# cover-vla/cover-vla

Hardware: AMD Instinct MI355X
Metric: candidate actions scored/sec (whole node), OpenVLA-7B N=32, 224^2 RGB (higher is better)
Workload: dtype bf16; 1 GPU; OpenVLA-7B (DINOv2-L+SigLIP-So400m+Llama-2-7B) N=32 = 8 prompts x 4 samples per GPU, 7 action tokens, 1 224x224 RGB frame(s); CoVer verifier SigLIP2-L/16-384 + 3-member ensemble; random-init weights with decision margins (depth-scaled residual projections, unit-scale embeddings, log-normal gains on the action rows of the head: synth.openvla_state(peaked=True)); candidates_total=32, candidates_per_gpu=32, prompts_per_gpu=8, parallelism=candidate-sharded x1 (weak), own_kv=legacy

## Files before the change

cover_vla_amd/_lib.py:

```python
from __future__ import annotations

import ctypes as C
import os

import torch

_HERE = os.path.dirname(os.path.abspath(__file__))
LIB_PATH = os.environ.get("COVER_LIB_PATH") or os.path.join(_HERE, "libcover_hip.so")

c_p = C.c_void_p
c_ll = C.c_longlong
c_i = C.c_int
c_f = C.c_float


class CoverError(RuntimeError):
    pass


class GemmEpi(C.Structure):
    _fields_ = [("bias", c_p), ("residual", c_p), ("layer_scale", c_p), ("ld_residual", c_i), ("residual_f32", c_i),
                ("act", c_i), ("glu", c_i), ("out_f32", c_i), ("out_scale", c_f),
                ("norm_w", c_p), ("norm_out", c_p), ("ld_norm_out", c_i), ("norm_style", c_i), ("norm_w_offset", c_f),
                ("norm_eps", c_f), ("norm_b", c_p), ("w8", c_p), ("w8_scale", c_p), ("a8", c_p), ("a8_scale", c_p), ("ld_a8", c_i), ("ld_norm_out8", c_i),
                ("norm_out8", c_p), ("norm_out8_scale", c_p),
                ("a8_mx", c_p), ("out8", c_p), ("out8_mx", c_p), ("ld_out8", c_i), ("w8_klinear", c_i)]


class KvSegment(C.Structure):
    _fields_ = [("k", c_p), ("vt", c_p),
                ("k_slot_stride", c_ll), ("k_t_stride", c_ll), ("k_h_stride", c_ll),
                ("vt_slot_stride", c_ll), ("vt_h_stride", c_ll), ("vt_d_stride", c_ll),
                ("slot_of_batch", c_p), ("len_of_batch", c_p), ("vis_len", c_p),
                ("len", c_i), ("mask_mode", c_i), ("causal_offset", c_i), ("_pad", c_i)]


class AttnArgs(C.Structure):
    _fields_ = [("q", c_p), ("out", c_p),
                ("q_b_stride", c_ll), ("q_t_stride", c_ll), ("q_h_stride", c_ll),
                ("o_b_stride", c_ll), ("o_t_stride", c_ll), ("o_h_stride", c_ll),
                ("B", c_i), ("Tq", c_i), ("Hq", c_i), ("Hkv", c_i), ("D", c_i), ("scale", c_f),
                ("n_seg", c_i), ("_pad", c_i), ("seg", KvSegment * 3),
                ("state_in_o", c_p), ("state_in_ml", c_p), ("state_out_o", c_p), ("state_out_ml", c_p),
                ("out8", c_p), ("out8_mx", c_p), ("out8_rows", c_i), ("_pad2", c_i)]


class DecodeAttnArgs(C.Structure):
    _fields_ = [("qkv", c_p), ("ld_qkv", c_i), ("n_splits", c_i), ("partial", c_p), ("bias", c_p),
                ("N", c_i), ("H", c_i), ("D", c_i), ("scale", c_f),
                ("positions", c_p), ("cos_table", c_p), ("sin_table", c_p), ("n_pos", c_i), ("rope_mode", c_i),
                ("seg", KvSegment * 3), ("write_t", c_i), ("_pad", c_i), ("out", c_p), ("out_row_stride", c_ll)]


class OwnAttnArgs(C.Structure):
    _fields_ = [("qkv", c_p), ("ld_qkv", c_i), ("N", c_i), ("H", c_i), ("D", c_i), ("scale", c_f),
                ("positions", c_p), ("cos_table", c_p), ("sin_table", c_p), ("n_pos", c_i), ("rope_mode", c_i),
                ("k", c_p), ("v", c_p), ("k_scale", c_p), ("v_scale", c_p), ("fp8", c_i), ("t_cap", c_i),
                ("slot_stride", c_ll), ("slot_of_batch", c_p), ("write_t", c_i), ("_pad", c_i),
                ("state_o", c_p), ("state_ml", c_p)]


class RopeArgs(C.Structure):
    _fields_ = [("qkv", c_p), ("ld_qkv", c_i),
                ("B", c_i), ("T", c_i), ("Hq", c_i), ("Hkv", c_i), ("D", c_i),
                ("positions", c_p), ("cos_table", c_p), ("sin_table", c_p), ("n_pos", c_i),
                ("rope_mode", c_i),
                ("k_cache", c_p), ("k_slot_stride", c_ll), ("k_t_stride", c_ll), ("k_h_stride", c_ll),
                ("vt_cache", c_p), ("vt_slot_stride", c_ll), ("vt_h_stride", c_ll), ("vt_d_stride", c_ll),
                ("slot_of_batch", c_p), ("t_offset_of_batch", c_p), ("t_offset", c_i), ("n_splits", c_i),
                ("partial", c_p), ("bias", c_p)]


class PatchifyArgs(C.Structure):
    _fields_ = [("img", c_p), ("in_u8_hwc", c_i), ("H", c_i), ("W", c_i), ("patch", c_i), ("n_img", c_i),
                ("img_stride", c_ll), ("mul", c_f * 3), ("add", c_f * 3), ("out", c_p), ("ld_out", c_i)]


class GemmF32Args(C.Structure):
    _fields_ = [("A", c_p), ("a_row_stride", c_ll), ("a_k_stride", c_ll),
                ("B", c_p), ("b_row_stride", c_ll), ("b_k_stride", c_ll),
                ("C", c_p), ("c_row_stride", c_ll),
                ("bias", c_p), ("residual", c_p), ("ld_residual", c_ll),
                ("M", c_i), ("N", c_i), ("K", c_i), ("act", c_i), ("alpha", c_f),
                ("batch", c_i), ("a_batch_stride", c_ll), ("b_batch_stride", c_ll), ("c_batch_stride", c_ll),
                ("bias_batch_stride", c_ll)]


class MhaF32Args(C.Structure):
    _fields_ = [("q", c_p), ("q_b_stride", c_ll), ("q_t_stride", c_ll),
                ("k", c_p), ("k_b_stride", c_ll), ("k_t_stride", c_ll),
                ("v", c_p), ("v_b_stride", c_ll), ("v_t_stride", c_ll),
                ("out", c_p), ("o_b_stride", c_ll), ("o_t_stride", c_ll),
                ("key_pad", c_p), ("B", c_i), ("Tq", c_i), ("Tk", c_i), ("H", c_i), ("Dh", c_i), ("scale", c_f)]


class TokenSelectArgs(C.Structure):
    _fields_ = [("logits", c_p), ("ld", c_ll), ("rows", c_i), ("lo", c_i), ("hi", c_i),
                ("uniform", c_p), ("temperature", c_f), ("token_out", c_p), ("logit_out", c_p)]


class TokenSampleArgs(C.Structure):
    _fields_ = [("logits", c_p), ("ld", c_ll), ("rows", c_i), ("lo", c_i), ("hi", c_i),
                ("uniform", c_p), ("temperature", c_f), ("top_k", c_i), ("top_p", c_f),
                ("token_out", c_p), ("logit_out", c_p), ("kept_out", c_p)]


class TokenSampleScoredArgs(C.Structure):
    _fields_ = TokenSampleArgs._fields_ + [("logprob_out", c_p)]

# ... 106 lines not shown
                ("cum_out", c_p), ("step_lp_out", c_p), ("g_out", c_p), ("kappa_out", c_p)]


class Workspace(C.Structure):
    _fields_ = [("ptr", c_p), ("bytes", C.c_size_t)]


class VitLayer(C.Structure):
    _fields_ = [("ln1_w", c_p), ("ln1_b", c_p), ("ln2_w", c_p), ("ln2_b", c_p),
                ("qkv_w", c_p), ("qkv_b", c_p), ("proj_w", c_p), ("proj_b", c_p),
                ("fc1_w", c_p), ("fc1_b", c_p), ("fc2_w", c_p), ("fc2_b", c_p), ("ls1", c_p), ("ls2", c_p)]


class VitDesc(C.Structure):
    _fields_ = [("dim", c_i), ("heads", c_i), ("head_dim_p", c_i), ("mlp_p", c_i), ("n_layers", c_i), ("act", c_i),
                ("ln_eps", c_f), ("attn_scale", c_f), ("layers_host", C.POINTER(VitLayer)),
                ("last_attn_only", c_i), ("_pad", c_i)]


class DecLayer(C.Structure):
    _fields_ = [("in_norm_w", c_p), ("post_norm_w", c_p), ("qkv_w", c_p), ("qkv_b", c_p), ("o_w", c_p),
                ("gate_up_w", c_p), ("down_w", c_p), ("k_cache", c_p), ("vt_cache", c_p),
                ("qkv_w8", c_p), ("qkv_s", c_p), ("o_w8", c_p), ("o_s", c_p), ("gate_up_w8", c_p), ("gate_up_s", c_p),
                ("down_w8", c_p), ("down_s", c_p), ("down_klinear", c_i), ("o_klinear", c_i)]


class DecDesc(C.Structure):
    _fields_ = [("dim", c_i), ("Hq", c_i), ("Hkv", c_i), ("D", c_i), ("mlp", c_i), ("n_layers", c_i), ("act", c_i),
                ("norm_style", c_i), ("norm_eps", c_f), ("norm_w_offset", c_f), ("attn_scale", c_f),
                ("rope_mode", c_i), ("n_pos", c_i), ("_pad", c_i),
                ("cos_table", c_p), ("sin_table", c_p), ("final_norm_w", c_p),
                ("layers_host", C.POINTER(DecLayer))]


class DecGroup(C.Structure):
    _fields_ = [("B", c_i), ("T", c_i), ("positions", c_p), ("n_seg", c_i), ("write_seg", c_i),
                ("segs", KvSegment * 3), ("seg_k_offset", c_ll * 3), ("seg_vt_offset", c_ll * 3),
                ("write_slot_of_batch", c_p), ("write_t_offset_of_batch", c_p),
                ("write_t_offset", c_i), ("seg0_shared", c_i),
                ("own_kv_mode", c_i), ("seg1_group", c_i), ("seg1_slot_of_group", c_p), ("seg1_len_of_group", c_p),
                ("own_region_elems", c_ll)]


class DecPass(C.Structure):
    _fields_ = [("n_groups", c_i), ("final_norm", c_i), ("x_f32", c_p), ("groups", DecGroup * 2)]


_STRUCTS = {
    "cover_gemm_epi": GemmEpi, "cover_kv_segment": KvSegment, "cover_attn_args": AttnArgs,
    "cover_rope_args": RopeArgs, "cover_patchify_args": PatchifyArgs, "cover_gemm_f32_args": GemmF32Args,
    "cover_mha_f32_args": MhaF32Args, "cover_token_select_args": TokenSelectArgs,
    "cover_token_sample_args": TokenSampleArgs, "cover_token_sample_scored_args": TokenSampleScoredArgs,
    "cover_token_logprob_args": TokenLogprobArgs, "cover_token_topn_args": TokenTopnArgs,
    "cover_token_sample_rows_args": TokenSampleRowsArgs, "cover_token_logprob_rows_args": TokenLogprobRowsArgs,
    "cover_token_topn_rows_args": TokenTopnRowsArgs, "cover_token_allow": TokenAllow, "cover_token_ref": TokenRef, "cover_decode_feedback_args": DecodeFeedbackArgs,
    "cover_token_fsm": TokenFsm,
    "cover_score_select_args": ScoreSelectArgs, "cover_prior_select_args": PriorSelectArgs, "cover_augment_args": AugmentArgs,
    "cover_proposal_prior_args": ProposalPriorArgs,
    "cover_beam_merge_args": BeamMergeArgs,
    "cover_kv_gather_slots_args": KvGatherSlotsArgs, "cover_beam_backtrack_args": BeamBacktrackArgs,
    "cover_gumbel_topn_args": GumbelTopnArgs, "cover_beam_merge_gumbel_args": BeamMergeGumbelArgs, "cover_workspace": Workspace, "cover_vit_layer": VitLayer,
    "cover_vit_desc": VitDesc, "cover_dec_layer": DecLayer, "cover_dec_desc": DecDesc, "cover_dec_group": DecGroup,
    "cover_dec_pass": DecPass, "cover_decode_attn_args": DecodeAttnArgs, "cover_own_attn_args": OwnAttnArgs,
}

_P = C.POINTER
SYMBOLS = {
    "cover_abi_version": (c_i, []),
    "cover_last_error": (C.c_char_p, []),
    "cover_device_info": (c_i, [c_i, _P(c_i), _P(C.c_size_t), C.c_char_p, c_i]),
    "cover_packed_weight_bytes": (C.c_size_t, [c_i, c_i]),
    "cover_packed_k": (c_i, [c_i]),
    "cover_pack_weight_bf16": (c_i, [c_p, c_i, c_i, c_i, c_p, c_i, c_p]),
    "cover_packed_weight_fp8_bytes": (C.c_size_t, [c_i, c_i]),
    "cover_quantize_rows_fp8": (c_i, [c_p, c_i, c_i, c_i, c_p, c_p, c_p]),
    "cover_pack_weight_fp8": (c_i, [c_p, c_i, c_p, c_i, c_i, c_p, c_p, c_i, c_p]),
    "cover_quantize_act_fp8": (c_i, [c_p, c_i, c_i, c_i, c_p, c_i, c_p, c_p]),
    "cover_quantize_act_fp8_mx": (c_i, [c_p, c_i, c_i, c_i, c_p, c_i, c_p, c_p]),
    "cover_pack_weight_fp8_klinear": (c_i, [c_p, c_i, c_p, c_i, c_i, c_p, c_p, c_p]),
    "cover_gemm_workspace_bytes": (C.c_size_t, [c_i, c_i, c_i]),
    "cover_gemm_bf16": (c_i, [c_p, c_i, c_p, c_p, c_i, c_i, c_i, c_i, _P(GemmEpi), c_p, C.c_size_t, c_i, c_p]),
    "cover_gemm_plan_counts": (c_i, [C.POINTER(C.c_longlong), c_i, c_i]),
    "cover_gemm_plan": (c_i, [c_p, c_i, c_p, c_p, c_i, c_i, c_i, c_i, _P(GemmEpi), c_p, C.c_size_t, c_i, C.POINTER(c_i)]),
    "cover_gemm_probe": (c_i, [C.POINTER(C.c_ulonglong)]),
    "cover_attention_bf16": (c_i, [_P(AttnArgs), c_p]),
    "cover_attention_plan": (c_i, [_P(AttnArgs), _P(c_i)]),
    "cover_attention_bf16_pair": (c_i, [_P(AttnArgs), _P(AttnArgs), c_p]),
    "cover_attention_pair_plan": (c_i, [_P(AttnArgs), _P(AttnArgs), _P(c_i)]),
    "cover_decode_attention_fused": (c_i, [_P(DecodeAttnArgs), c_p]),
    "cover_decode_own_attention": (c_i, [_P(OwnAttnArgs), c_p]),
    "cover_layernorm_bf16": (c_i, [c_p, c_i, c_p, c_p, c_p, c_i, c_i, c_i, c_f, c_p]),
    "cover_rmsnorm_bf16": (c_i, [c_p, c_i, c_i, c_p, c_f, c_i, c_p, c_i, c_i, c_i, c_f, c_p]),
    "cover_rmsnorm_bf16_q8": (c_i, [c_p, c_i, c_i, c_p, c_f, c_i, c_p, c_i, c_i, c_i, c_f, c_p, c_i, c_p, c_p]),
    "cover_rope_kv_write": (c_i, [_P(RopeArgs), c_p]),
    "cover_rope_kv_write_pair": (c_i, [_P(RopeArgs), _P(RopeArgs), c_p]),
    "cover_embed_gather": (c_i, [c_p, c_i, c_p, c_i, c_f, c_p, c_i, c_p]),
    "cover_patchify": (c_i, [_P(PatchifyArgs), c_p]),
    "cover_copy_rows_bf16": (c_i, [c_p, c_i, c_p, c_i, c_i, c_i, c_p, c_p, c_p]),
    "cover_add_rows_bf16": (c_i, [c_p, c_i, c_p, c_i, c_i, c_i, c_i, c_p]),
    "cover_scale_bf16": (c_i, [c_p, c_i, c_i, c_i, c_f, c_f, c_p]),
    "cover_cast_f32_to_bf16": (c_i, [c_p, c_i, c_p, c_i, c_i, c_i, c_p]),
    "cover_cast_bf16_to_f32": (c_i, [c_p, c_i, c_p, c_i, c_i, c_i, c_p]),
    "cover_gemm_f32": (c_i, [_P(GemmF32Args), c_p]),
    "cover_gemm_f32_plan": (c_i, [_P(GemmF32Args), _P(c_i)]),
    "cover_layernorm_f32": (c_i, [c_p, c_i, c_p, c_p, c_p, c_i, c_i, c_i, c_f, c_p]),
    "cover_layernorm_f32_grouped": (c_i, [c_p, c_i, c_p, c_p, c_p, c_i, c_i, c_i, c_f, c_i, c_ll, c_p]),
    "cover_softmax_rows_f32": (c_i, [c_p, c_i, c_i, c_i, c_f, c_p]),
    "cover_l2norm_rows_f32": (c_i, [c_p, c_i, c_p, c_i, c_i, c_i, c_p]),
    "cover_add_f32": (c_i, [c_p, c_i, c_p, c_i, c_p, c_i, c_i, c_i, c_i, c_p]),
    "cover_xent_diag_f32": (c_i, [c_p, c_i, c_i, c_i, c_p, c_p, c_p]),
    "cover_act_f32": (c_i, [c_p, c_i, c_p, c_i, c_i, c_i, c_i, c_p]),
    "cover_mha_f32": (c_i, [_P(MhaF32Args), c_p]),
    "cover_masked_mean_f32": (c_i, [c_p, c_p, c_p, c_i, c_i, c_i, c_p]),
    "cover_sincos_time_embed": (c_i, [c_p, c_i, c_i, C.c_double, C.c_double, c_p, c_i, c_p]),
    "cover_token_select": (c_i, [_P(TokenSelectArgs), c_p]),
    "cover_token_sample": (c_i, [_P(TokenSampleArgs), c_p]),
    "cover_token_sample_scored": (c_i, [_P(TokenSampleScoredArgs), c_p]),
    "cover_token_logprob": (c_i, [_P(TokenLogprobArgs), c_p]),
    "cover_token_topn": (c_i, [_P(TokenTopnArgs), c_p]),
    "cover_token_sample_rows": (c_i, [_P(TokenSampleRowsArgs), c_p]),
    "cover_token_logprob_rows": (c_i, [_P(TokenLogprobRowsArgs), c_p]),
    "cover_token_topn_rows": (c_i, [_P(TokenTopnRowsArgs), c_p]),
    "cover_token_sample_rows_allowed": (c_i, [_P(TokenSampleRowsArgs), _P(TokenAllow), c_p]),
    "cover_token_logprob_rows_allowed": (c_i, [_P(TokenLogprobRowsArgs), _P(TokenAllow), c_p]),
    "cover_token_topn_rows_allowed": (c_i, [_P(TokenTopnRowsArgs), _P(TokenAllow), c_p]),
    "cover_token_sample_rows_ref": (c_i, [_P(TokenSampleRowsArgs), _P(TokenAllow), _P(TokenRef), c_p]),
    "cover_decode_feedback": (c_i, [_P(DecodeFeedbackArgs), c_p]),
    "cover_decode_feedback_lp2": (c_i, [_P(DecodeFeedbackArgs), c_p, c_p, c_ll, c_p]),
    "cover_decode_feedback_fsm": (c_i, [_P(DecodeFeedbackArgs), _P(TokenFsm), c_p, c_p, c_ll, c_p]),
    "cover_score_select": (c_i, [_P(ScoreSelectArgs), c_p]),
    "cover_group_argmax": (c_i, [c_p, c_i, c_i, c_p, c_p, c_p]),
    "cover_prior_select": (c_i, [_P(PriorSelectArgs), c_p]),
    "cover_augment_tokens": (c_i, [_P(AugmentArgs), c_p]),
    "cover_augment_actions": (c_i, [_P(AugmentArgs), c_p]),
    "cover_proposal_prior_tokens": (c_i, [_P(ProposalPriorArgs), c_p]),
    "cover_proposal_prior_actions": (c_i, [_P(ProposalPriorArgs), c_p]),
    "cover_beam_merge": (c_i, [_P(BeamMergeArgs), c_p]),
    "cover_kv_gather_slots": (c_i, [_P(KvGatherSlotsArgs), c_p]),
    "cover_beam_backtrack": (c_i, [_P(BeamBacktrackArgs), c_p]),
    "cover_gumbel_topn": (c_i, [_P(GumbelTopnArgs), c_p]),
    "cover_beam_merge_gumbel": (c_i, [_P(BeamMergeGumbelArgs), c_p]),
    "cover_tokens_to_histories": (c_i, [c_p, c_i, c_i, c_i, c_p, c_i, c_p, c_i, c_f, c_p, c_p, c_p]),
    "cover_tokens_to_histories_steps": (c_i, [c_p, c_i, c_i, c_i, c_p, c_i, c_p, c_i, c_i, c_f, c_p, c_p, c_p]),
    "cover_actions_to_histories": (c_i, [c_p, c_ll, c_ll, c_i, c_i, c_p, c_p, c_i, c_f, c_p, c_p, c_p]),
    "cover_resample_axis": (c_i, [c_p, c_i, c_p, c_i, c_i, c_i, c_i, c_i, c_i, c_i, c_p, c_p, c_i, c_i, c_p]),
    "cover_u8_hwc_to_f32_chw_norm": (c_i, [c_p, c_p, c_i, c_i, _P(c_f), _P(c_f), c_p]),
    "cover_u8_hwc_to_f32_chw_scale_norm": (c_i, [c_p, c_p, c_i, c_i, c_f, _P(c_f), _P(c_f), c_p]),
    "cover_resize_bilinear_pad_f32": (c_i, [c_p, c_p, c_i, c_i, c_i, c_i, c_i, c_i, c_i, c_i, c_i, c_f, c_p]),
    "cover_vit_workspace_bytes": (C.c_size_t, [_P(VitDesc), c_i, c_i]),
    "cover_vit_forward": (c_i, [_P(VitDesc), c_p, c_i, c_i, c_p, Workspace, c_i, c_p]),
    "cover_decoder_workspace_bytes": (C.c_size_t, [_P(DecDesc), c_i]),
    "cover_decoder_forward": (c_i, [_P(DecDesc), _P(DecPass), c_p, Workspace, c_i, c_p]),
    "cover_graph_begin": (c_i, [c_p]),
    "cover_graph_end": (c_i, [c_p, _P(c_p)]),
    "cover_graph_launch": (c_i, [c_p, c_p]),
    "cover_graph_destroy": (c_i, [c_p]),
    "cover_timer_create": (c_i, [_P(c_p)]),
    "cover_timer_start": (c_i, [c_p, c_p]),
    "cover_timer_stop": (c_i, [c_p, c_p, _P(c_f)]),
    "cover_timer_destroy": (c_i, [c_p]),
    "cover_stream_sync": (c_i, [c_p]),
    "cover_profile_begin": (c_i, [c_i]),
    "cover_profile_end": (c_i, [_P(C.c_double), _P(C.c_longlong), _P(C.c_double)]),
    "cover_profile_end_n": (c_i, [_P(C.c_double), _P(C.c_longlong), _P(C.c_double), c_i]),
    "cover_sizeof": (C.c_size_t, [C.c_char_p]),
}
# ... 38 lines not shown
```

cover_vla_amd/csrc/capi.hip:

```cpp
#include <hip/hip_runtime.h>
#include <stdio.h>
#include <stdlib.h>
#include <string.h>
#include <string>
#include "kernels.h"

static thread_local std::string g_err;
int fail(int code, const char* what, hipError_t e) {
    char buf[512];
    if (e != hipSuccess) snprintf(buf, sizeof buf, "%s: %s", what, hipGetErrorString(e));
    else snprintf(buf, sizeof buf, "%s", what);
    g_err = buf;
    return code;
}
#define ST(s) ((hipStream_t)(s))

extern "C" {

int cover_abi_version(void) { return COVER_ABI_VERSION; }
const char* cover_last_error(void) { return g_err.c_str(); }

int cover_device_info(int dev, int* n_cu, size_t* total_mem, char* name, int name_len) {
    hipDeviceProp_t p;
    HIPCHK(hipGetDeviceProperties(&p, dev), "hipGetDeviceProperties");
    if (n_cu) *n_cu = p.multiProcessorCount;
    if (total_mem) *total_mem = p.totalGlobalMem;
    if (name && name_len > 0) {
        strncpy(name, p.gcnArchName, name_len - 1);
        name[name_len - 1] = 0;
    }
    return COVER_OK;
}

int cover_packed_k(int K) { return (K + 127) / 128 * 128; }
size_t cover_packed_weight_bytes(int N, int K) {
    return (size_t)((N + 15) / 16) * 16 * (size_t)cover_packed_k(K) * 2;
}
int cover_pack_weight_bf16(const void* W, int ldw, int N, int K, void* Wp, int glu, void* stream) {
    if (!W || !Wp || N <= 0 || K <= 0) return fail(COVER_EINVAL, "cover_pack_weight_bf16: bad arguments");
    if (glu && ((N / 2) % 16 != 0 || (N & 1))) return fail(COVER_EINVAL, "cover_pack_weight_bf16: glu needs N/2 % 16 == 0");
    HIPCHK(launch_pack_weight_bf16((const bf16_t*)W, ldw, N, K, (bf16_t*)Wp, cover_packed_k(K), glu, ST(stream)),
           "pack_weight");
    return COVER_OK;
}
size_t cover_packed_weight_fp8_bytes(int N, int K) { return (size_t)((N + 15) / 16) * 16 * (size_t)cover_packed_k(K); }
int cover_quantize_rows_fp8(const void* W, int ldw, int N, int K, float* scales, void* Wdq, void* stream) {
    if (!W || !scales || !Wdq || N <= 0 || K <= 0) return fail(COVER_EINVAL, "cover_quantize_rows_fp8: bad arguments");
    HIPCHK(launch_quantize_rows_fp8((const bf16_t*)W, ldw, N, K, scales, (bf16_t*)Wdq, ST(stream)), "quantize_rows_fp8");
    return COVER_OK;
}
int cover_pack_weight_fp8(const void* Wdq, int ldw, const float* scales, int N, int K, void* Wq, float* scales_packed, int glu,
                          void* stream) {
    if (!Wdq || !scales || !Wq || !scales_packed || N <= 0 || K <= 0) return fail(COVER_EINVAL, "cover_pack_weight_fp8: bad arguments");
    if (glu && ((N / 2) % 16 != 0 || (N & 1))) return fail(COVER_EINVAL, "cover_pack_weight_fp8: glu needs N/2 % 16 == 0");
    HIPCHK(launch_pack_weight_fp8((const bf16_t*)Wdq, ldw, scales, N, K, (uint8_t*)Wq, scales_packed, cover_packed_k(K), glu, ST(stream)),
           "pack_weight_fp8");
    return COVER_OK;
}
int cover_pack_weight_fp8_klinear(const void* Wdq, int ldw, const float* scales, int N, int K, void* Wq, float* scales_packed, void* stream) {
    if (!Wdq || !scales || !Wq || !scales_packed || N <= 0 || K <= 0) return fail(COVER_EINVAL, "cover_pack_weight_fp8_klinear: bad arguments");
    HIPCHK(launch_pack_weight_fp8((const bf16_t*)Wdq, ldw, scales, N, K, (uint8_t*)Wq, scales_packed, cover_packed_k(K), 0, ST(stream), 1),
           "pack_weight_fp8 (k-linear)");
    return COVER_OK;
}
int cover_quantize_act_fp8_mx(const void* X, int ldx, int M, int K, void* out8, int ld8, void* mx, void* stream) {
    if (!X || !out8 || !mx || M < 0 || K <= 0) return fail(COVER_EINVAL, "cover_quantize_act_fp8_mx: bad arguments");
    HIPCHK(launch_quantize_act_fp8_mx((const bf16_t*)X, ldx, M, K, (uint8_t*)out8, ld8, (uint8_t*)mx, ST(stream)),
           "quantize_act_fp8_mx (ld8 >= padded K, ld8 % 16 == 0, ldx % 8 == 0)");
    return COVER_OK;
}
int cover_quantize_act_fp8(const void* X, int ldx, int M, int K, void* out8, int ld8, float* scales, void* stream) {
    if (!X || !out8 || !scales || M < 0 || K <= 0) return fail(COVER_EINVAL, "cover_quantize_act_fp8: bad arguments");
    HIPCHK(launch_quantize_act_fp8((const bf16_t*)X, ldx, M, K, (uint8_t*)out8, ld8, scales, ST(stream)),
           "quantize_act_fp8 (ld8 >= padded K, ld8 % 16 == 0, ldx % 8 == 0)");
    return COVER_OK;
}
size_t cover_gemm_workspace_bytes(int M, int N, int K) { return gemm_workspace_bytes(M, N, K); }
int cover_gemm_probe(unsigned long long* out) {
    if (!out) return fail(COVER_EINVAL, "cover_gemm_probe: null pointer");
    if (gemm_v3_probe(out) != 0) return fail(COVER_EHIP, "cover_gemm_probe: could not read the probe words");
    return COVER_OK;
}
int cover_gemm_plan_counts(long long* counts, int n, int reset) {
    if (n < 0 || (n > 0 && !counts)) return fail(COVER_EINVAL, "cover_gemm_plan_counts: bad arguments");
    gemm_plan_counts(counts, n, reset);
    return COVER_GEMM_PLANS;
}
static const char* gemm_args_error(const void* A, int lda, const void* Wp, const void* C, int N, int K, const cover_gemm_epi* epi) {
    if (!A || !Wp || !C) return "cover_gemm_bf16: null pointer";
    if (lda % 8) return "cover_gemm_bf16: lda must be a multiple of 8 elements";
    if (lda < cover_packed_k(K)) return "cover_gemm_bf16: lda < padded K";
    if (epi && epi->glu && (N % 32)) return "cover_gemm_bf16: glu needs N % 32 == 0";
    return nullptr;
}
int cover_gemm_plan(const void* A, int lda, const void* Wp, void* C, int ldc, int M, int N, int K,
                    const cover_gemm_epi* epi, void* ws, size_t ws_bytes, int variant, int plan[6]) {
    if (!plan) return fail(COVER_EINVAL, "cover_gemm_plan: null plan");
    if (const char* why = gemm_args_error(A, lda, Wp, C, N, K, epi)) return fail(COVER_EINVAL, why);
    HIPCHK(gemm_plan_query((const bf16_t*)A, lda, (const bf16_t*)Wp, C, ldc, M, N, K, epi, (const float*)ws, ws_bytes, variant, plan), "gemm_plan");
    return COVER_OK;
}
int cover_gemm_bf16(const void* A, int lda, const void* Wp, void* C, int ldc, int M, int N, int K,
                    const cover_gemm_epi* epi, void* ws, size_t ws_bytes, int variant, void* stream) {
    if (const char* why = gemm_args_error(A, lda, Wp, C, N, K, epi)) return fail(COVER_EINVAL, why);
    HIPCHK(launch_gemm_bf16((const bf16_t*)A, lda, (const bf16_t*)Wp, C, ldc, M, N, K, epi, (float*)ws, ws_bytes, variant,
                            ST(stream)),
           "gemm_bf16");
    return COVER_OK;
}

int cover_attention_bf16(const cover_attn_args* a, void* stream) {
    if (!a) return fail(COVER_EINVAL, "cover_attention_bf16: null args");
    HIPCHK(launch_attention_bf16(a, ST(stream)), "attention_bf16 (D must be 64/96/128/256, 1..3 segments)");
    return COVER_OK;
}

int cover_attention_plan(const cover_attn_args* a, int* plan) {
    if (!a || !plan) return fail(COVER_EINVAL, "cover_attention_plan: null pointer");
    HIPCHK(attention_plan(a, plan), "attention_bf16 (D must be 64/96/128/256, 1..3 segments)");
    return COVER_OK;
}
int cover_attention_bf16_pair(const cover_attn_args* a0, const cover_attn_args* a1, void* stream) {
    if (!a0 || !a1) return fail(COVER_EINVAL, "cover_attention_bf16_pair: null args");
    HIPCHK(launch_attention_bf16_pair(a0, a1, ST(stream)), "attention_bf16_pair (D must be 64/96/128/256, 1..3 segments)");
    return COVER_OK;
}
int cover_attention_pair_plan(const cover_attn_args* a0, const cover_attn_args* a1, int* dual) {
    if (!a0 || !a1 || !dual) return fail(COVER_EINVAL, "cover_attention_pair_plan: null pointer");
    HIPCHK(attention_pair_plan(a0, a1, dual), "attention_bf16_pair (D must be 64/96/128/256, 1..3 segments)");
    return COVER_OK;
}
int cover_decode_attention_fused(const cover_decode_attn_args* a, void* stream) {
    if (!a || !a->out || (a->n_splits <= 0 && !a->qkv) || (a->n_splits > 0 && !a->partial))
        return fail(COVER_EINVAL, "cover_decode_attention_fused: null pointer");
    HIPCHK(launch_decode_attention_fused(a, ST(stream)), "decode_attention_fused (D in {64,128}, COVER_MASK_LEN segments, 0 <= write_t < seg[2].len)");
    return COVER_OK;
}

int cover_decode_own_attention(const cover_own_attn_args* a, void* stream) {
    if (!a) return fail(COVER_EINVAL, "cover_decode_own_attention: null args");
    HIPCHK(launch_decode_own_attention(a, ST(stream)), "decode_own_attention (D in {64,128}, 0 <= write_t < t_cap, at most 16 loads per lane per pass)");
    return COVER_OK;
}

int cover_layernorm_bf16(const void* x, int ldx, const float* w, const float* b, void* y, int ldy, int rows, int dim,
                         float eps, void* stream) {
    HIPCHK(launch_layernorm_bf16((const bf16_t*)x, ldx, w, b, (bf16_t*)y, ldy, rows, dim, eps, ST(stream)), "layernorm_bf16");
    return COVER_OK;
}
int cover_rmsnorm_bf16(const void* x, int x_f32, int ldx, const float* w, float w_offset, int style, void* y, int ldy,
                       int rows, int dim, float eps, void* stream) {
    HIPCHK(launch_rmsnorm(x, x_f32, ldx, w, w_offset, style, (bf16_t*)y, ldy, rows, dim, eps, ST(stream)), "rmsnorm_bf16");
    return COVER_OK;
}
int cover_rmsnorm_bf16_q8(const void* x, int x_f32, int ldx, const float* w, float w_offset, int style, void* y, int ldy,
                          int rows, int dim, float eps, void* q8, int ld8, float* q8s, void* stream) {
    if (!q8 || !q8s) return fail(COVER_EINVAL, "cover_rmsnorm_bf16_q8: null q8 / q8s");
    HIPCHK(launch_rmsnorm(x, x_f32, ldx, w, w_offset, style, (bf16_t*)y, ldy, rows, dim, eps, ST(stream), (uint8_t*)q8, ld8, q8s), "rmsnorm_bf16_q8");
    return COVER_OK;
}
int cover_rope_kv_write(const cover_rope_args* a, void* stream) {
    if (!a) return fail(COVER_EINVAL, "cover_rope_kv_write: null args");
    HIPCHK(launch_rope_kv_write(a, ST(stream)), "rope_kv_write");
    return COVER_OK;
}
int cover_rope_kv_write_pair(const cover_rope_args* a0, const cover_rope_args* a1, void* stream) {
    if (!a0 || !a1) return fail(COVER_EINVAL, "cover_rope_kv_write_pair: null args");
    HIPCHK(launch_rope_kv_write_pair(a0, a1, ST(stream)), "rope_kv_write_pair");
    return COVER_OK;
}
int cover_embed_gather(const void* table, int dim, const int64_t* ids, int n, float scale, void* out, int ldo,
                       void* stream) {
    HIPCHK(launch_embed_gather((const bf16_t*)table, dim, ids, n, scale, (bf16_t*)out, ldo, ST(stream)), "embed_gather");
    return COVER_OK;
}
int cover_patchify(const cover_patchify_args* a, void* stream) {
    if (!a || a->patch <= 0 || a->H % a->patch || a->W % a->patch || a->ld_out < 3 * a->patch * a->patch)
        return fail(COVER_EINVAL, "cover_patchify: bad geometry");
    HIPCHK(launch_patchify(a, ST(stream)), "patchify");
    return COVER_OK;
}
int cover_copy_rows_bf16(const void* src, int ld_src, void* dst, int ld_dst, int rows, int cols, const int* sidx,
// ... 364 lines not shown
```

cover_vla_amd/csrc/gemm_bf16.hip:

```cpp
#include <stdlib.h>
#include <string.h>
#include <atomic>
#include <hip/hip_ext.h>
#include "common.h"
#include "kernels.h"

#ifdef COVER_PC_DEBUG
__device__ unsigned long long g_pc_tl[1024 * 8];
#define PCTL(slot) do { if (threadIdx.x == 0) g_pc_tl[((blockIdx.y * gridDim.x + blockIdx.x) & 1023) * 8 + (slot)] = wall_clock64(); } while (0)
#else
#define PCTL(slot) do { } while (0)
#endif

#include "gemm_common.h"



template <int WM, int WN, bool GLDS, int NST_ = 2, int WGM = 2, int WGN = 2>
__global__ __launch_bounds__(64 * WGM * WGN) void gemm_tiled(const bf16_t* __restrict__ A, int lda,
                                                  const bf16_t* __restrict__ Wp, void* C, int ldc, int M, int N,
                                                  int Kp, EpiDev epi, int tiles_m, int tiles_n, int kt_per,
                                                  float* __restrict__ partial) {
    constexpr int NW = WGM * WGN;
    constexpr int BM_ = WGM * WM * 16, BN_ = WGN * WN * 16;
// ... 567 lines not shown
#pragma unroll
        for (int c = 0; c < 2; ++c)
            if ((int)(threadIdx.x + c * 512) * 8 < N)
#pragma unroll
                for (int i = 0; i < 8; ++i) sum += vals[c][i];
        mean = block_sum_lds(sum, red) / N;
        float q2 = 0.f;
#pragma unroll
        for (int c = 0; c < 2; ++c)
            if ((int)(threadIdx.x + c * 512) * 8 < N)
#pragma unroll
                for (int i = 0; i < 8; ++i) {
                    const float d = vals[c][i] - mean;
                    q2 += d * d;
                }
        rstd = rsqrtf(block_sum_lds(q2, red + 8) / N + epi.norm_eps);
    } else {
        RNT(3);
        rstd = rsqrtf(block_sum_lds(q, red) / N + epi.norm_eps);
        RNT(4);
    }
#pragma unroll
    for (int c = 0; c < 2; ++c) {
        const int n0 = (threadIdx.x + c * 512) * 8;
        if (n0 < N) {
            float o[8];
            const float wv[8] = {nw[c][0].x, nw[c][0].y, nw[c][0].z, nw[c][0].w, nw[c][1].x, nw[c][1].y, nw[c][1].z, nw[c][1].w};
#pragma unroll
            for (int i = 0; i < 8; ++i) {
                const float ww = wv[i];
                if (epi.norm_style == 2) o[i] = (vals[c][i] - mean) * rstd * ww + (epi.norm_b ? epi.norm_b[n0 + i] : 0.f);
                else o[i] = epi.norm_style == 1 ? ww * bfround(vals[c][i] * rstd) : vals[c][i] * rstd * (epi.norm_w_offset + ww);
            }
            uint4 u;
            u.x = pack_bf2(o[0], o[1]); u.y = pack_bf2(o[2], o[3]); u.z = pack_bf2(o[4], o[5]); u.w = pack_bf2(o[6], o[7]);
            *(uint4*)(epi.norm_out + (size_t)m * epi.ld_norm_out + n0) = u;
            if (epi.nq8) {
#pragma unroll
                for (int i = 0; i < 8; ++i) vals[c][i] = bfround(o[i]);
            }
        }
    }
    if (epi.nq8) {
        float mx = 0.f;
#pragma unroll
        for (int c = 0; c < 2; ++c)
            if ((int)(threadIdx.x + c * 512) * 8 < N)
#pragma unroll
                for (int i = 0; i < 8; ++i) mx = fmaxf(mx, fabsf(vals[c][i]));
        mx = wave_max(mx);
        if ((threadIdx.x & 63) == 0) red[8 + (threadIdx.x >> 6)] = mx;
        asm volatile("s_waitcnt lgkmcnt(0)\n\ts_barrier" ::: "memory");
        float t = 0.f;
#pragma unroll
        for (int i = 0; i < 8; ++i) t = fmaxf(t, red[8 + i]);
        const float sc = e4m3_pow2_scale(t), inv = 1.0f / sc;
        if (threadIdx.x == 0) epi.nq8s[m] = sc;
        uint8_t* qrow = epi.nq8 + (size_t)m * epi.ldnq8;
#pragma unroll
        for (int c = 0; c < 2; ++c) {
            const int n0 = (threadIdx.x + c * 512) * 8;
            if (n0 < N) store_q8_chunk(qrow, n0, vals[c], inv);
        }
    }
    RNT(5);
}
__global__ __launch_bounds__(512) void splitk_reduce_norm(const float* __restrict__ partial, int S, bf16_t* C, int ldc, int M,
                                                          int N, EpiDev epi) {
    __shared__ float red[16];
    reduce_norm_row(partial, S, C, ldc, M, N, epi, blockIdx.x, red);
}

__device__ __forceinline__ void slab_store4(float* o, const float (&v)[4], int n, int N) {
    if (n + 3 < N && ((((uintptr_t)o) & 15) == 0)) {
        *(float4*)o = make_float4(v[0], v[1], v[2], v[3]);
    } else {
        for (int e = 0; e < 4; ++e)
            if (n + e < N) o[e] = v[e];
    }
}

template <int MF, int KS, int NBW, bool W8 = false>
__global__ __launch_bounds__(512) void gemm_skinny2(const bf16_t* __restrict__ A, int lda, const bf16_t* __restrict__ Wp,
                                                    float* __restrict__ partial, int M, int N, int Kp, const float* __restrict__ wscale, int kl) {
    constexpr int NG = 8 / KS, KC = 256 * KS, NBPB = NG * NBW;
    extern __shared__ __attribute__((aligned(16))) char smem[];
    const int tid = threadIdx.x, lane = tid & 63;
    const int w = __builtin_amdgcn_readfirstlane(tid >> 6);
    const int ks = w % KS, ng = w / KS;
    const int s = blockIdx.y;
    const int k0 = s * KC;
    const int kc = min(KC, Kp - k0);
    const int K32 = Kp >> 5;
    const int N16 = (N + 15) >> 4;
    const int nb_begin = blockIdx.x * NBPB;
    const int kw0 = ks * 256;
    const int nsteps = max(0, min(8, (kc - kw0) >> 5));
    f32x4 acc[NBW][MF];
#pragma unroll
    for (int i = 0; i < NBW; ++i)
#pragma unroll
        for (int f = 0; f < MF; ++f) acc[i][f] = (f32x4){0.f, 0.f, 0.f, 0.f};
    constexpr int NLD = W8 ? 4 : 8;
    auto wsrc = [&](int nb, int k) -> const u32x4* {
        if constexpr (W8) return (const u32x4*)((const uint8_t*)Wp + ((size_t)nb * (Kp >> 6) + (k >> 6)) * 1024) + lane;
        else return (const u32x4*)(Wp + ((size_t)nb * K32 + (k >> 5)) * 512) + lane;
    };
    u32x4 buf[2][NLD];
    auto load8 = [&](u32x4(&dst)[NLD], int i) {
        int nb = nb_begin + ng + NG * i;
        nb = nb < N16 ? nb : N16 - 1;
        const u32x4* src = wsrc(nb, k0 + kw0);
        if (nsteps == 8) {
#pragma unroll
            for (int u = 0; u < NLD; ++u) dst[u] = __builtin_nontemporal_load(src + u * 64);
        } else {
#pragma unroll
            for (int u = 0; u < NLD; ++u)
                if (u * (8 / NLD) < nsteps) dst[u] = __builtin_nontemporal_load(src + u * 64);
        }
    };
    constexpr int NFR = (KC / 32) * MF;
    bool items_done = false;
    if (kc == KC && nsteps == 8 && NBW > 1) {
        constexpr int XL = NFR / 8;
        uint4 xr[XL];
        const int rr = lane & 15, gg = lane >> 4;
#pragma unroll
        for (int j = 0; j < XL; ++j) {
            const int fi = j * 8 + w, kst = fi / MF, f = fi - kst * MF;
            int row = f * 16 + rr;
            row = row < M ? row : M - 1;
            xr[j] = *(const uint4*)(A + (size_t)row * lda + k0 + x_run_k<W8>(kst, gg, kl));
        }
#pragma unroll
        for (int i = 0; i < 2; ++i) {
            int nb = nb_begin + ng + NG * i;
            nb = nb < N16 ? nb : N16 - 1;
            const u32x4* src = wsrc(nb, k0 + kw0);
#pragma unroll
            for (int u = 0; u < NLD; ++u) buf[i][u] = __builtin_nontemporal_load(src + u * 64);
        }
#pragma unroll
        for (int j = 0; j < XL; ++j) *(uint4*)(smem + (j * 8 + w) * 1024 + lane * 16) = xr[j];
        asm volatile("s_waitcnt lgkmcnt(0)\n\ts_barrier" ::: "memory");
#pragma unroll
        for (int i = 0; i < NBW; ++i) {
#pragma unroll
            for (int u = 0; u < 8; ++u) {
                const bf16x8 wf = wfrag<W8>(buf[i & 1], u);
                const int kst = (kw0 >> 5) + u;
#pragma unroll
                for (int f = 0; f < MF; ++f) {
                    const bf16x8 xf = as_bf16x8(*(const uint4*)(smem + ((kst * MF + f) * 64 + lane) * 16));
                    acc[i][f] = __builtin_amdgcn_mfma_f32_16x16x32_bf16(wf, xf, acc[i][f], 0, 0, 0);
                }
            }
            __builtin_amdgcn_sched_barrier(0);
            if (i + 2 < NBW) {
                int nb = nb_begin + ng + NG * (i + 2);
                nb = nb < N16 ? nb : N16 - 1;
                const u32x4* src = wsrc(nb, k0 + kw0);
#pragma unroll
                for (int u = 0; u < NLD; ++u) buf[i & 1][u] = __builtin_nontemporal_load(src + u * 64);
                __builtin_amdgcn_sched_barrier(0);
            }
        }
        items_done = true;
    } else {
        load8(buf[0], 0);
        if (NBW > 1) load8(buf[1], 1);
        {
            const int rr = lane & 15, gg = lane >> 4;
#pragma unroll 4
            for (int fi = w; fi < NFR; fi += 8) {
                const int kst = fi / MF, f = fi - kst * MF;
                const int row = f * 16 + rr, kk = x_run_k<W8>(kst, gg, kl);
                uint4 v = make_uint4(0, 0, 0, 0);
                if (row < M && kk < kc) v = *(const uint4*)(A + (size_t)row * lda + k0 + kk);
                *(uint4*)(smem + fi * 1024 + lane * 16) = v;
            }
        }
        __syncthreads();
    }
    auto comp8 = [&](u32x4(&src)[NLD], f32x4(&a)[MF]) {
        auto step = [&](int u) {
            const bf16x8 wf = wfrag<W8>(src, u);
            const int kst = (kw0 >> 5) + u;
#pragma unroll
            for (int f = 0; f < MF; ++f) {
                const bf16x8 xf = as_bf16x8(*(const uint4*)(smem + ((kst * MF + f) * 64 + lane) * 16));
                a[f] = __builtin_amdgcn_mfma_f32_16x16x32_bf16(wf, xf, a[f], 0, 0, 0);
            }
        };
        if (nsteps == 8) {
#pragma unroll
            for (int u = 0; u < 8; ++u) step(u);
        } else {
#pragma unroll
            for (int u = 0; u < 8; ++u)
                if (u < nsteps) step(u);
        }
    };
    if (!items_done) {
#pragma unroll
        for (int i = 0; i < NBW; ++i) {
            comp8(buf[i & 1], acc[i]);
            if (i + 2 < NBW) load8(buf[i & 1], i + 2);
        }
    }
    constexpr int RB = (8 / MF) < NBW ? (8 / MF) : NBW;
    const int r = lane & 15, g = lane >> 4;
    float* red = (float*)smem;
#pragma unroll
    for (int i0 = 0; i0 < NBW; i0 += RB) {
        __syncthreads();
#pragma unroll
        for (int ii = 0; ii < RB; ++ii)
            if (i0 + ii < NBW) {
#pragma unroll
                for (int f = 0; f < MF; ++f)
#pragma unroll
                    for (int e = 0; e < 4; ++e) red[(((w * RB + ii) * MF + f) * 4 + e) * 64 + lane] = acc[(i0 + ii) < NBW ? (i0 + ii) : 0][f][e];
            }
        __syncthreads();
        constexpr int NFRAG = NG * RB * MF;
        for (int j = w; j < NFRAG; j += 8) {
            const int f = j % MF, ii = (j / MF) % RB, gsel = j / (MF * RB);
            if (i0 + ii >= NBW) continue;
            const int nb = nb_begin + gsel + NG * (i0 + ii);
            float v[4] = {0.f, 0.f, 0.f, 0.f};
#pragma unroll
            for (int kk = 0; kk < KS; ++kk) {
                const int ww = gsel * KS + kk;
#pragma unroll
                for (int e = 0; e < 4; ++e) v[e] += red[(((ww * RB + ii) * MF + f) * 4 + e) * 64 + lane];
            }
            const int m = f * 16 + r, n = nb * 16 + 4 * g;
            if constexpr (W8) {
                const float4 sc = *(const float4*)(wscale + (size_t)(nb < N16 ? nb : N16 - 1) * 16 + 4 * g);
                v[0] *= sc.x; v[1] *= sc.y; v[2] *= sc.z; v[3] *= sc.w;
            }
            if (nb < N16 && m < M && n < N) slab_store4(partial + ((size_t)s * M + m) * N + n, v, n, N);
        }
    }
}

#ifdef COVER_SK_DEBUG
__device__ unsigned long long g_sk_dbg[1024 * 4];
extern "C" int cover_sk_debug(unsigned long long* out) {
    return (int)hipMemcpyFromSymbol(out, HIP_SYMBOL(g_sk_dbg), sizeof(g_sk_dbg));
}
#define SKT(slot) do { if (threadIdx.x == 0) g_sk_dbg[((blockIdx.y * gridDim.x + blockIdx.x) & 1023) * 4 + (slot)] = wall_clock64(); } while (0)
#else
#define SKT(slot) do { } while (0)
#endif
template <int MF, int KS, int NBW, int NBUF, bool W8 = false>
__global__ __launch_bounds__(512) void gemm_skinny3(const bf16_t* __restrict__ A, int lda, const bf16_t* __restrict__ Wp,
                                                    void* C, int ldc, int M, int N, int Kp, EpiDev epi,
                                                    float* __restrict__ partial, int kper, const float* __restrict__ wscale, int kl) {
    SKT(0);
    constexpr int NG = 8 / KS, KC = 256 * KS, NBPB = NG * NBW;
    constexpr int XB = MF * 16 * KC * 2;
    constexpr int XL = XB / (512 * 16);
    extern __shared__ __attribute__((aligned(16))) char smem[];
    const int tid = threadIdx.x, lane = tid & 63;
    const int w = __builtin_amdgcn_readfirstlane(tid >> 6);
    const int ks = w % KS, ng = w / KS;
    const int K32 = Kp >> 5;
    const int N16 = (N + 15) >> 4;
    const int nb_begin = blockIdx.x * NBPB;
    const int kb = blockIdx.y * kper;
    const int ke = min(Kp, kb + kper);
    const int nchunks = (ke - kb + KC - 1) / KC;
    const int kw0 = ks * 256;
    f32x4 acc[NBW][MF];
#pragma unroll
    for (int i = 0; i < NBW; ++i)
#pragma unroll
        for (int f = 0; f < MF; ++f) acc[i][f] = (f32x4){0.f, 0.f, 0.f, 0.f};

    const int items = nchunks * NBW;
    auto steps_of = [&](int c) { return max(0, min(8, (min(KC, ke - kb - c * KC) - kw0) >> 5)); };
    constexpr int NLD = W8 ? 4 : 8;
    auto wsrc = [&](int nb, int k) -> const u32x4* {
        if constexpr (W8) return (const u32x4*)((const uint8_t*)Wp + ((size_t)nb * (Kp >> 6) + (k >> 6)) * 1024) + lane;
        else return (const u32x4*)(Wp + ((size_t)nb * K32 + (k >> 5)) * 512) + lane;
    };
    u32x4 buf[NBUF][NLD];
    auto load8 = [&](u32x4(&dst)[NLD], int t) {
        const int c = t / NBW, i = t - c * NBW;
        int nb = nb_begin + ng + NG * i;
        nb = nb < N16 ? nb : N16 - 1;
        const int nst = steps_of(c);
        const u32x4* src = wsrc(nb, kb + c * KC + kw0);
        if (nst == 8) {
#pragma unroll
            for (int u = 0; u < NLD; ++u) dst[u] = __builtin_nontemporal_load(src + u * 64);
        } else {
#pragma unroll
            for (int u = 0; u < NLD; ++u)
                if (u * (8 / NLD) < nst) dst[u] = __builtin_nontemporal_load(src + u * 64);
        }
    };
    static_assert(XL * 8 == (KC / 32) * MF, "fragments must split evenly over the waves");
    uint4 xr[XL];
    const int srr = lane & 15, sgg = lane >> 4;
    auto x_load = [&](int c) {
        const int k0 = kb + c * KC, kc = min(KC, ke - k0);
#pragma unroll
        for (int j = 0; j < XL; ++j) {
            const int fi = j * 8 + w, kst = fi / MF, f = fi - kst * MF;
            const int row = f * 16 + srr, kk = x_run_k<W8>(kst, sgg, kl);
            xr[j] = make_uint4(0, 0, 0, 0);
            if (row < M && kk < kc) xr[j] = *(const uint4*)(A + (size_t)row * lda + k0 + kk);
        }
    };
    auto x_write = [&](int b) {
#pragma unroll
        for (int j = 0; j < XL; ++j) *(uint4*)(smem + b * XB + (j * 8 + w) * 1024 + lane * 16) = xr[j];
    };
    auto comp8 = [&](u32x4(&src)[NLD], f32x4(&a)[MF], int c) {
        const int nst = steps_of(c);
        const char* xb = smem + (c & 1) * XB;
        auto step = [&](int u) {
            const bf16x8 wf = wfrag<W8>(src, u);
            const int kst = (kw0 >> 5) + u;
#pragma unroll
            for (int f = 0; f < MF; ++f) {
                const bf16x8 xf = as_bf16x8(*(const uint4*)(xb + ((kst * MF + f) * 64 + lane) * 16));
                a[f] = __builtin_amdgcn_mfma_f32_16x16x32_bf16(wf, xf, a[f], 0, 0, 0);
            }
        };
        if (nst == 8) {
#pragma unroll
            for (int u = 0; u < 8; ++u) step(u);
        } else {
#pragma unroll
            for (int u = 0; u < 8; ++u)
                if (u < nst) step(u);
        }
    };

    if (items >= NBUF && min(KC, ke - kb) == KC) {
        {
#pragma unroll
            for (int j = 0; j < XL; ++j) {
                const int fi = j * 8 + w, kst = fi / MF, f = fi - kst * MF;
                int row = f * 16 + srr;
                row = row < M ? row : M - 1;
                xr[j] = *(const uint4*)(A + (size_t)row * lda + kb + x_run_k<W8>(kst, sgg, kl));
            }
        }
#pragma unroll
// ... 74 lines not shown
    }
    int t = c0 * NBW;
    for (int c = c0; c < nchunks; ++c) {
        if (c + 1 < nchunks) x_load(c + 1);
#pragma unroll
        for (int i = 0; i < NBW; ++i, ++t) {
            comp8(buf[i % NBUF], acc[i], c);
            if (t + NBUF < items) load8(buf[i % NBUF], t + NBUF);
        }
        if (c + 1 < nchunks) {
            x_write((c + 1) & 1);
            asm volatile("s_waitcnt lgkmcnt(0)\n\ts_barrier" ::: "memory");
        }
    }

    SKT(2);
    constexpr int RB = (8 / MF) < NBW ? (8 / MF) : NBW;
    const int r = lane & 15, g = lane >> 4;
    float* red = (float*)smem;
#pragma unroll
    for (int i0 = 0; i0 < NBW; i0 += RB) {
        __syncthreads();
#pragma unroll
        for (int ii = 0; ii < RB; ++ii)
            if (i0 + ii < NBW) {
#pragma unroll
                for (int f = 0; f < MF; ++f)
#pragma unroll
                    for (int e = 0; e < 4; ++e) red[(((w * RB + ii) * MF + f) * 4 + e) * 64 + lane] = acc[(i0 + ii) < NBW ? (i0 + ii) : 0][f][e];
            }
        __syncthreads();
        auto slice_sum = [&](int gsel, int ii, int f, float (&v)[4]) {
#pragma unroll
            for (int e = 0; e < 4; ++e) v[e] = 0.f;
#pragma unroll
            for (int kk = 0; kk < KS; ++kk) {
                const int ww = gsel * KS + kk;
#pragma unroll
                for (int e = 0; e < 4; ++e) v[e] += red[(((ww * RB + ii) * MF + f) * 4 + e) * 64 + lane];
            }
            if constexpr (W8) {
                const int nbs = nb_begin + gsel + NG * (i0 + ii);
                const float4 sc = *(const float4*)(wscale + (size_t)(nbs < N16 ? nbs : N16 - 1) * 16 + 4 * g);
                v[0] *= sc.x; v[1] *= sc.y; v[2] *= sc.z; v[3] *= sc.w;
            }
        };
        if (partial) {
            constexpr int NFRAG = NG * RB * MF;
            for (int j = w; j < NFRAG; j += 8) {
                const int f = j % MF, ii = (j / MF) % RB, gsel = j / (MF * RB);
                if (i0 + ii >= NBW) continue;
                const int nb = nb_begin + gsel + NG * (i0 + ii);
                const int m = f * 16 + r, n = nb * 16 + 4 * g;
                if (nb < N16 && m < M && n < N) {
                    float v[4];
                    slice_sum(gsel, ii, f, v);
                    slab_store4(partial + ((size_t)blockIdx.y * M + m) * N + n, v, n, N);
                }
            }
        } else if (epi.glu) {
            constexpr int NFRAG = RB * MF;
            for (int j = w; j < NFRAG; j += 8) {
                const int f = j % MF, ii = j / MF;
                if (i0 + ii >= NBW) continue;
                const int nb = nb_begin + NG * (i0 + ii);
                const int m = f * 16 + r;
                if (nb + 1 < N16 + (N16 & 1) && nb < N16 && m < M) {
                    float gv[4], uv[4];
                    slice_sum(0, ii, f, gv);
                    slice_sum(1, ii, f, uv);
                    epi_store4_glu(epi, C, ldc, m, (nb >> 1) * 16 + 4 * g, N >> 1, gv, uv);
                }
            }
        } else {
            constexpr int NFRAG = NG * RB * MF;
            for (int j = w; j < NFRAG; j += 8) {
                const int f = j % MF, ii = (j / MF) % RB, gsel = j / (MF * RB);
                if (i0 + ii >= NBW) continue;
                const int nb = nb_begin + gsel + NG * (i0 + ii);
                const int m = f * 16 + r;
                if (nb < N16 && m < M) {
                    float v[4];
                    slice_sum(gsel, ii, f, v);
                    epi_store4(epi, C, ldc, m, nb * 16 + 4 * g, N, v);
                }
            }
        }
    }
    SKT(3);
}

__global__ __launch_bounds__(256) void splitk_reduce(const float* __restrict__ partial, int S, void* C, int ldc, int M,
                                                     int N, EpiDev epi) {
    const int Nout = epi.glu ? (N >> 1) : N;
    const int groups = (Nout + 3) >> 2;
    const long long total = (long long)M * groups;
    for (long long idx = (long long)blockIdx.x * blockDim.x + threadIdx.x; idx < total;
         idx += (long long)gridDim.x * blockDim.x) {
        const int m = (int)(idx / groups);
        const int j0 = (int)(idx - (long long)m * groups) * 4;
        if (epi.glu) {
            const int ng = (j0 >> 4) * 32 + (j0 & 15);
            float gv[4] = {0, 0, 0, 0}, uv[4] = {0, 0, 0, 0};
            for (int s = 0; s < S; ++s) {
                const float* p = partial + ((size_t)s * M + m) * N + ng;
#pragma unroll
                for (int i = 0; i < 4; ++i)
                    if (j0 + i < Nout) {
                        gv[i] += p[i];
                        uv[i] += p[16 + i];
                    }
            }
            epi_store4_glu(epi, C, ldc, m, j0, Nout, gv, uv);
        } else {
            float v[4] = {0, 0, 0, 0};
            const float* p0 = partial + (size_t)m * N + j0;
            const size_t sstride = (size_t)M * N;
            if (j0 + 3 < N && ((((uintptr_t)p0) | (sstride * sizeof(float))) & 15) == 0) {
                int s = 0;
                for (; s + 4 <= S; s += 4) {
                    float4 a[4];
#pragma unroll
                    for (int j = 0; j < 4; ++j) a[j] = *(const float4*)(p0 + (s + j) * sstride);
#pragma unroll
                    for (int j = 0; j < 4; ++j) { v[0] += a[j].x; v[1] += a[j].y; v[2] += a[j].z; v[3] += a[j].w; }
                }
                for (; s < S; ++s) {
                    const float4 a = *(const float4*)(p0 + s * sstride);
                    v[0] += a.x; v[1] += a.y; v[2] += a.z; v[3] += a.w;
                }
            } else {
                for (int s = 0; s < S; ++s) {
                    const float* p = partial + ((size_t)s * M + m) * N + j0;
#pragma unroll
                    for (int i = 0; i < 4; ++i)
                        if (j0 + i < N) v[i] += p[i];
                }
            }
            epi_store4(epi, C, ldc, m, j0, N, v);
        }
    }
}


__global__ void pack_weight(const bf16_t* __restrict__ W, int ldw, int N, int K, bf16_t* __restrict__ Wp, int Kp,
                            int glu) {
    const int K32 = Kp >> 5;
    const int N16 = (N + 15) >> 4;
    const long long total = (long long)N16 * K32 * 64;
    for (long long idx = (long long)blockIdx.x * blockDim.x + threadIdx.x; idx < total;
         idx += (long long)gridDim.x * blockDim.x) {
        const int lane = (int)(idx & 63);
        const long long blk = idx >> 6;
        const int kb = (int)(blk % K32);
        const int nb = (int)(blk / K32);
        int n = nb * 16 + (lane & 15);
        if (glu) {
            const int half = N >> 1;
            const int i = nb >> 1;
            n = ((nb & 1) ? half : 0) + i * 16 + (lane & 15);
            if (i * 16 + (lane & 15) >= half) n = N;
        }
        const int k = kb * 32 + (lane >> 4) * 8;
        bf16_t v[8];
#pragma unroll
        for (int e = 0; e < 8; ++e) v[e] = (n < N && k + e < K) ? W[(size_t)n * ldw + k + e] : (bf16_t)0;
        *(uint4*)(Wp + idx * 8) = *(const uint4*)v;
    }
}

static EpiDev make_epi(const cover_gemm_epi* e) {
    EpiDev d;
    d.bias = e ? e->bias : nullptr;
    d.residual = e ? e->residual : nullptr;
    d.res_f32 = e ? e->residual_f32 : 0;
    d.lscale = e ? e->layer_scale : nullptr;
    d.ldr = e ? e->ld_residual : 0;
    d.act = e ? e->act : 0;
    d.glu = e ? e->glu : 0;
    d.out_f32 = e ? e->out_f32 : 0;
    d.out_scale = e ? e->out_scale : 1.0f;
    if (d.out_scale == 0.0f) d.out_scale = 1.0f;
    d.norm_w = e ? e->norm_w : nullptr;
    d.norm_b = e ? e->norm_b : nullptr;
    d.norm_out = e ? (bf16_t*)e->norm_out : nullptr;
    d.ld_norm_out = e ? e->ld_norm_out : 0;
    d.norm_style = e ? e->norm_style : 0;
    d.norm_w_offset = e ? e->norm_w_offset : 0.f;
    d.norm_eps = e ? e->norm_eps : 0.f;
    d.w8 = e ? (const uint8_t*)e->w8 : nullptr;
    d.w8s = e ? e->w8_scale : nullptr;
    if (!d.w8 || !d.w8s) { d.w8 = nullptr; d.w8s = nullptr; }
    d.a8 = e ? (const uint8_t*)e->a8 : nullptr;
    d.a8s = e ? e->a8_scale : nullptr;
    d.lda8 = e ? e->ld_a8 : 0;
    if (!d.a8 || !d.a8s || !d.w8) { d.a8 = nullptr; d.a8s = nullptr; }
    d.nq8 = e ? (uint8_t*)e->norm_out8 : nullptr;
    d.nq8s = e ? e->norm_out8_scale : nullptr;
    d.ldnq8 = e ? e->ld_norm_out8 : 0;
    if (!d.nq8 || !d.nq8s || !d.norm_out || d.norm_style == 2) { d.nq8 = nullptr; d.nq8s = nullptr; }
    d.w8_kl = (e && d.w8) ? e->w8_klinear : 0;
    d.a8mx = (e && d.w8 && e->a8) ? (const uint8_t*)e->a8_mx : nullptr;
    if (d.a8mx) { d.a8 = (const uint8_t*)e->a8; d.a8s = nullptr; }
    d.o8 = e ? (uint8_t*)e->out8 : nullptr;
    d.o8mx = e ? (uint8_t*)e->out8_mx : nullptr;
    d.ldo8 = e ? e->ld_out8 : 0;
    if (!d.o8 || !d.o8mx) { d.o8 = nullptr; d.o8mx = nullptr; }
    return d;
}

static inline int sk_class(int N, int K) { return 2.0 * (double)N * (double)K >= 16.0e6 ? 0 : 3; }

static Skinny3Plan plan_skinny3(int M, int N, int Kp) {
    Skinny3Plan best;
    best.ok = false;
    best.MF = (M + 15) / 16;
    const int N16 = (N + 15) / 16;
    if (M > 32 || (N16 & 1) || Kp < 2048) return best;
    int best_blocks = 0;
    const int nbws[3] = {4, 3, 2};
    for (int bi = 0; bi < 3; ++bi) {
        const int nbw = nbws[bi];
        const int gx = (N16 + 2 * nbw - 1) / (2 * nbw);
        for (int S = 1; S <= 8; ++S) {
            if ((long long)gx * S > 256) break;
            const int kraw = (Kp + S - 1) / S;
            int kper = (kraw + 1023) / 1024 * 1024;
            if ((long long)kper * (S - 1) >= Kp) kper = (kraw + 255) / 256 * 256;
            if (kper < 2048) break;
            if ((long long)kper * (S - 1) >= Kp) continue;
            const int blocks = gx * S;
            if (blocks > best_blocks) {
                best_blocks = blocks;
                best.ok = true; best.NBW = nbw; best.S = S; best.kper = kper; best.gx = gx;
            }
        }
    }
    if (!best.ok || best_blocks < 190) { best.ok = false; return best; }
    best.lds = (size_t)2 * best.MF * 16 * 1024 * 2;
    best.ws_bytes = best.S > 1 ? (size_t)best.S * M * N * sizeof(float) : 0;
    return best;
}

static SkinnyPlan plan_skinny(int M, int N, int Kp) {
    SkinnyPlan p;
    p.MF = (M + 15) / 16;
    const int N16 = (N + 15) / 16;
    p.nbpb = N16 >= 1024 ? 16 : 8;
    p.gx = (N16 + p.nbpb - 1) / p.nbpb;
    const int kc_max = (64 * 1024) / (p.MF * 16 * 2) / 128 * 128;
    int S = (512 + p.gx - 1) / p.gx;
    int kb = Kp / 128;
    if (S > kb) S = kb;
    if (S < 1) S = 1;
    int KC = ((kb + S - 1) / S) * 128;
    if (KC > kc_max) KC = kc_max;
    p.KC = KC;
    p.S = (Kp + KC - 1) / KC;
    p.lds = (size_t)p.MF * 16 * KC * 2;
    p.ws_bytes = (size_t)p.S * M * N * sizeof(float);
    return p;
}

static Skinny2Plan plan_skinny2(int M, int N, int Kp) {
    Skinny2Plan p;
    p.MF = (M + 15) / 16;
    p.KS = p.MF <= 2 ? 4 : 2;
    const int KC = 256 * p.KS, NG = 8 / p.KS;
    p.S = (Kp + KC - 1) / KC;
    const int N16 = (N + 15) / 16;
    static const char* slots_env = getenv("COVER_SK_SLOTS");
    const int slots = slots_env ? atoi(slots_env) : 512;
    if (p.MF <= 2) {
        const int cand[4] = {2, 3, 4, 6};
        p.NBW = 4;
        bool found = false;
        for (int c = 0; c < 4 && !found; ++c) {
            const long long blocks = (long long)((N16 + NG * cand[c] - 1) / (NG * cand[c])) * p.S;
            if (blocks <= slots) { p.NBW = cand[c]; found = true; }
        }
    } else {
        p.NBW = 2;
    }
    p.gx = (N16 + NG * p.NBW - 1) / (NG * p.NBW);
    const int rb = (8 / p.MF) < p.NBW ? (8 / p.MF) : p.NBW;
    const size_t x = (size_t)p.MF * 16 * KC * 2, red = (size_t)8 * rb * p.MF * 4 * 64 * 4;
    p.lds = x > red ? x : red;
    p.ws_bytes = (size_t)p.S * M * N * sizeof(float);
    return p;
}
// ... 139 lines not shown
    if (mx_any) {
        if (!f8_on) return hipErrorInvalidValue;
        if (pick != TP_PC_256x128 && pick != TP_PC_128x256 && pick != TP_PC_224x128 && pick != TP_PC_128x192 && !(pick == TP_PC_64x128 && epi.a8mx && !epi.o8))
            pick = TP_PC_128x256;
    }
    if (!(f8_on && gemm_fp8_tiled_supported(pick)) && ((pick >= TP_PC_128x128 && pick <= TP_PC_128x192) || pick == TP_PC_64x128_S3)) pick = (variant == 2 || pick == TP_PC_64x128_S3) ? TP_64x128 : TP_128x128;
    if (variant == 2 && pick > TP_64x64) pick = TP_128x128;
    const bool f8 = f8_on && gemm_fp8_tiled_supported(pick);
    const TileCfg cd = k_tiles[pick];
    const int bm = cd.wm * cd.wgm * 16, bn = cd.wn * cd.wgn * 16;
    p.pick = pick;
    p.tiles_m = (M + bm - 1) / bm;
    p.tiles_n = (N + bn - 1) / bn;
    const int nk_total = Kp / BK;
    int S = 1;
    if (S_forced > 0 && !force) {
        S = S_forced;
    } else if (ws != nullptr) {
        while ((long long)p.tiles_m * p.tiles_n * S < 192 && S < 8 && nk_total / (S * 2) >= 8 && (size_t)(S * 2) * M * N * sizeof(float) <= ws_bytes)
            S *= 2;
        static const char* split_env = getenv("COVER_TILE_SPLIT");
        if (split_env && atoi(split_env) >= 1 && (size_t)atoi(split_env) * M * N * sizeof(float) <= ws_bytes) S = atoi(split_env);
    }
    if (epi.o8) S = 1;
    const int nst = variant == 2 ? 2 : cd.nst;
    p.lds = (size_t)nst * (bm + bn) * BK * 2;
    p.block = 64 * cd.wgm * cd.wgn;
    p.slot = pick;
    if (f8) {
        if (epi.lda8 < Kp || (epi.lda8 & 15)) return hipErrorInvalidValue;
        static const char* v3f8_env = getenv("COVER_V3_F8");
        const bool v3f8 = !(v3f8_env && v3f8_env[0] == '0') && (size_t)M * epi.lda8 + 4096 < ((size_t)1 << 31);
        p.kind = v3f8 && f8_self_loading(pick) ? GK_F8_V3 : GK_F8_PC;
        if (mx_any && p.kind != GK_F8_V3 && !(pick == TP_PC_64x128 && epi.a8mx && !epi.o8)) return hipErrorInvalidValue;
        if (epi.a8mx) p.lds += p.kind == GK_F8_V3 ? 3 * 1024 : 4 * 256;
        if (p.kind == GK_F8_PC) p.block += 256;
        p.slot = PLAN_FP8;
        const int nk8 = Kp / 128;
        p.kt_per = (nk8 + S - 1) / S;
        p.S = (nk8 + p.kt_per - 1) / p.kt_per;
        return hipSuccess;
    }
    p.kt_per = (nk_total + S - 1) / S;
    p.S = (nk_total + p.kt_per - 1) / p.kt_per;
    if (pick >= TP_V3_224x192) {
        if ((size_t)M * lda * 2 + 4096 >= ((size_t)1 << 31)) return hipErrorInvalidValue;
        p.kind = GK_V3;
        if (pick == TP_V3K_224x96) p.block *= 2;
    } else if (pick == TP_PC_64x128) {
        p.kind = GK_TILED_PC;
        p.block += 256;
    } else {
        p.kind = GK_TILED;
    }
    return hipSuccess;
}

static hipError_t plan_gemm(GemmPlan& p, int lda, const void* C, int ldc, int M, int N, int K, const EpiDev& epi, const float* ws, size_t ws_bytes,
                            int variant, bool want_slabs) {
    p = GemmPlan{};
    p.kind = GK_NONE; p.slot = -1; p.pick = -1;
    if (M <= 0 || N <= 0) return hipSuccess;
    const int Kp = (K + 127) / 128 * 128;
    if (variant == 0) variant = (M <= 64 && ws != nullptr) ? 3 : 1;
    const bool mx_any = epi.a8mx != nullptr || epi.o8 != nullptr;
    if (mx_any) {
        if (variant != 1 || !epi.a8 || !epi.w8 || M <= 64 || (size_t)M * epi.lda8 + 4096 >= ((size_t)1 << 31)) return hipErrorInvalidValue;
        if (epi.a8mx && (!epi.w8_kl || epi.glu)) return hipErrorInvalidValue;
        if (epi.o8 && (!epi.glu || (epi.act != ACT_SILU && epi.act != ACT_GELU_TANH) || ((N / 2) % 32) != 0 || epi.ldo8 < N / 2 || (epi.ldo8 & 15) || epi.out_f32))
            return hipErrorInvalidValue;
        if (epi.o8 && ((((uintptr_t)C) & 15) || (ldc % 8))) return hipErrorInvalidValue;
    }
    if (epi.w8_kl && epi.a8 && !epi.a8mx && M > 64) return hipErrorInvalidValue;
    hipError_t e;
    if (variant == 3 || variant == 6) e = plan_streaming(p, M, N, Kp, ws, ws_bytes, variant == 6, false);
    else if (variant == 5) {
        if (M > 64) return hipErrorInvalidValue;
        p.p1 = plan_skinny(M, N, Kp);
        if (ws == nullptr || ws_bytes < p.p1.ws_bytes) return hipErrorInvalidValue;
        p.kind = GK_SKINNY; p.slot = PLAN_SKINNY; p.S = p.p1.S; p.lds = p.p1.lds;
        e = hipSuccess;
    } else e = plan_tiles(p, lda, M, N, Kp, epi, ws, ws_bytes, variant, mx_any);
    if (e != hipSuccess) return e;
    const bool want_norm = epi.norm_w != nullptr && epi.norm_out != nullptr;
    const bool streaming = p.kind == GK_SKINNY || p.kind == GK_SKINNY2 || p.kind == GK_SKINNY3;
    const bool split = streaming ? !(p.kind == GK_SKINNY3 && p.S == 1) : p.S > 1;
    const bool norm_fusable = want_norm && !epi.glu && !epi.out_f32 && (N % 8) == 0 && N <= 8192 && (ldc % 8) == 0 && (epi.ld_norm_out % 8) == 0 &&
                              (((uintptr_t)epi.norm_w) & 15) == 0;
    p.rcls = streaming ? 5 : p.kind == GK_F8_PC || p.kind == GK_F8_V3 ? 9 : (double)N * (double)Kp >= 16.0e6 ? 8 : 6;
    if (!split) p.done = GD_NONE;
    else if (!streaming && want_slabs && !epi.residual && !epi.lscale && epi.act == ACT_NONE && epi.out_scale == 1.0f && !epi.glu && !epi.norm_out)
        p.done = GD_SLABS;
    else p.done = norm_fusable ? GD_REDUCE_NORM : GD_REDUCE;
    p.norm_launch = want_norm && p.done != GD_REDUCE_NORM;
    return hipSuccess;
}

hipError_t gemm_plan_query(const bf16_t* A, int lda, const bf16_t* Wp, const void* C, int ldc, int M, int N, int K, const cover_gemm_epi* epi_in,
                           const float* ws, size_t ws_bytes, int variant, int* plan) {
    GemmPlan p;
    const hipError_t e = plan_gemm(p, lda, C, ldc, M, N, K, make_epi(epi_in), ws, ws_bytes, variant, false);
    if (e != hipSuccess) return e;
    const int out[6] = {p.slot, p.pick, p.kind == GK_F8_V3 ? 1 : 0, p.S, p.done == GD_NONE ? 0 : p.done == GD_REDUCE ? 1 : 2, p.norm_launch ? 1 : 0};
    for (int i = 0; i < 6; ++i) plan[i] = out[i];
    return hipSuccess;
}

static hipError_t run_norm(const EpiDev& epi, void* C, int ldc, int M, int Nout, hipStream_t st) {
    if (epi.norm_style == 2)
        return launch_layernorm_bf16((const bf16_t*)C, ldc, epi.norm_w, epi.norm_b, epi.norm_out, epi.ld_norm_out, M, Nout, epi.norm_eps, st);
    return launch_rmsnorm(C, 0, ldc, epi.norm_w, epi.norm_w_offset, epi.norm_style, epi.norm_out, epi.ld_norm_out, M, Nout, epi.norm_eps, st,
                          epi.nq8, epi.ldnq8, epi.nq8s);
}

static hipError_t complete_splitk(const GemmPlan& p, const EpiDev& epi, const float* ws, void* C, int ldc, int M, int N, hipStream_t st) {
    hipError_t e = hipSuccess;
    if (p.done == GD_REDUCE_NORM) {
        e = launch_kernel<splitk_reduce_norm>(p.rcls, 0.0, dim3(M), dim3(512), 0, st, ws, p.S, (bf16_t*)C, ldc, M, N, epi);
    } else if (p.done == GD_REDUCE) {
        const int Nout = epi.glu ? N / 2 : N;
        const long long total = (long long)M * ((Nout + 3) / 4);
        int rb = (int)((total + 255) / 256);
        if (rb > 2048) rb = 2048;
        e = launch_kernel<splitk_reduce>(p.rcls, 0.0, dim3(rb), dim3(256), 0, st, ws, p.S, C, ldc, M, N, epi);
    }
    if (e == hipSuccess && p.done != GD_NONE) e = hipGetLastError();
    if (e == hipSuccess && p.norm_launch) e = run_norm(epi, C, ldc, M, epi.glu ? N / 2 : N, st);
    return e;
}

static hipError_t launch_skinny2(const Skinny2Plan& p, const bf16_t* A, int lda, const bf16_t* Wp, float* ws, int M, int N, int K, int Kp,
                                 const uint8_t* w8, const float* w8s, int kl, hipStream_t st) {
    const dim3 grid(p.gx, p.S), block(512);
    plan_hit(PLAN_SKINNY2);
#define SK2(MF_, KS_, NBW_, W8_) launch_kernel<gemm_skinny2<MF_, KS_, NBW_, W8_>>(sk_class(N, K), (W8_ ? 1.0 : 2.0) * (double)N * (double)K, grid, block, p.lds, st, \
                                                                                   A, lda, W8_ ? (const bf16_t*)w8 : Wp, ws, M, N, Kp, w8s, kl)
    hipError_t e;
    if (w8 && w8s && p.MF <= 2) {
        if (p.MF == 1) e = p.NBW == 6 ? SK2(1, 4, 6, true) : p.NBW == 4 ? SK2(1, 4, 4, true) : p.NBW == 3 ? SK2(1, 4, 3, true) : SK2(1, 4, 2, true);
        else e = p.NBW == 6 ? SK2(2, 4, 6, true) : p.NBW == 4 ? SK2(2, 4, 4, true) : p.NBW == 3 ? SK2(2, 4, 3, true) : SK2(2, 4, 2, true);
    } else {
        if (p.MF == 1) e = p.NBW == 6 ? SK2(1, 4, 6, false) : p.NBW == 4 ? SK2(1, 4, 4, false) : p.NBW == 3 ? SK2(1, 4, 3, false) : SK2(1, 4, 2, false);
        else if (p.MF == 2) e = p.NBW == 6 ? SK2(2, 4, 6, false) : p.NBW == 4 ? SK2(2, 4, 4, false) : p.NBW == 3 ? SK2(2, 4, 3, false) : SK2(2, 4, 2, false);
        else if (p.MF == 3) e = SK2(3, 2, 2, false);
        else e = SK2(4, 2, 2, false);
    }
#undef SK2
    if (e == hipSuccess) e = hipGetLastError();
    return e;
}

static hipError_t launch_skinny3(const Skinny3Plan& p, const bf16_t* A, int lda, const bf16_t* Wp, void* C, int ldc, int M, int N,
                                 int Kp, const EpiDev& epi, float* partial, hipStream_t st) {
    const dim3 grid(p.gx, p.S), block(512);
    plan_hit(PLAN_SKINNY3);
#define SK3(MF_, NBW_, W8_) launch_kernel<gemm_skinny3<MF_, 4, NBW_, NBW_, W8_>>(sk_class(N, Kp), (W8_ ? 1.0 : 2.0) * (double)N * (double)Kp, grid, block, p.lds, st, \
                                                                                  A, lda, W8_ ? (const bf16_t*)epi.w8 : Wp, C, ldc, M, N, Kp, epi, partial, p.kper, epi.w8s, epi.w8_kl)
    hipError_t e;
    if (epi.w8) {
        if (p.MF == 1) e = p.NBW == 4 ? SK3(1, 4, true) : p.NBW == 3 ? SK3(1, 3, true) : SK3(1, 2, true);
        else e = p.NBW == 4 ? SK3(2, 4, true) : p.NBW == 3 ? SK3(2, 3, true) : SK3(2, 2, true);
    } else {
        if (p.MF == 1) e = p.NBW == 4 ? SK3(1, 4, false) : p.NBW == 3 ? SK3(1, 3, false) : SK3(1, 2, false);
        else e = p.NBW == 4 ? SK3(2, 4, false) : p.NBW == 3 ? SK3(2, 3, false) : SK3(2, 2, false);
    }
#undef SK3
    if (e == hipSuccess) e = hipGetLastError();
    return e;
}

static hipError_t launch_tiles(const GemmPlan& p, const bf16_t* A, int lda, const bf16_t* Wp, void* C, int ldc, int M, int N, int K, int Kp,
                               const EpiDev& epi, float* partial, int variant, hipStream_t st) {
    const int tcls = (double)N * (double)Kp >= 16.0e6 ? 4 : 1;
    const double twork = 2.0 * (double)M * (double)N * (double)K;
    plan_hit(p.slot);
    if (p.kind == GK_F8_PC || p.kind == GK_F8_V3) return launch_gemm_fp8_tiled(p, epi, C, ldc, M, N, Kp, partial, twork, st);
    if (p.kind == GK_V3) {
        if (p.S == 1 && epi.out_f32 && !epi.bias && !epi.residual && !epi.lscale && epi.act == ACT_NONE && epi.out_scale == 1.0f && !epi.glu &&
            !epi.norm_out && ldc == N)
            partial = (float*)C;
        return launch_gemm_v3(p, A, lda, Wp, C, ldc, M, N, Kp, epi, partial, tcls, twork, st);
    }
    const dim3 grid(p.tiles_m * p.tiles_n, p.S), block(p.block);
#define T(KFN) launch_kernel<KFN>(tcls, twork, grid, block, p.lds, st, A, lda, Wp, C, ldc, M, N, Kp, epi, p.tiles_m, p.tiles_n, p.kt_per, partial)
    hipError_t e;
    if (p.kind == GK_TILED_PC) {
        e = T((gemm_tiled_pc<2, 4, 4, 4>));
    } else if (variant == 2) {
        e = p.pick == TP_128x128 ? T((gemm_tiled<4, 4, false, 2, 2, 2>)) : p.pick == TP_64x128 ? T((gemm_tiled<2, 4, false, 2, 2, 2>)) : T((gemm_tiled<2, 2, false, 2, 2, 2>));
    } else {
        switch (p.pick) {
            case TP_128x128: e = T((gemm_tiled<4, 4, true, 2, 2, 2>)); break;
            case TP_64x128: e = T((gemm_tiled<2, 4, true, 2, 2, 2>)); break;
            case TP_64x64: e = T((gemm_tiled<2, 2, true, 3, 2, 2>)); break;
            case TP_128x128_S4: e = T((gemm_tiled<4, 4, true, 4, 2, 2>)); break;
            case TP_256x128: e = T((gemm_tiled<4, 4, true, 3, 4, 2>)); break;
            case TP_128x256: e = T((gemm_tiled<4, 4, true, 3, 2, 4>)); break;
            case TP_64x128_S3: e = T((gemm_tiled<2, 4, true, 3, 2, 2>)); break;
            case TP_128x128_S3: e = T((gemm_tiled<4, 4, true, 3, 2, 2>)); break;
            default: e = T((gemm_tiled<2, 4, true, 4, 4, 2>)); break;
        }
    }
#undef T
    if (e == hipSuccess) e = hipGetLastError();
    return e;
}

hipError_t launch_gemm_bf16(const bf16_t* A, int lda, const bf16_t* Wp, void* C, int ldc, int M, int N, int K,
                            const cover_gemm_epi* epi_in, float* ws, size_t ws_bytes, int variant, hipStream_t st, int* splits_out) {
    if (splits_out) *splits_out = 0;
    const EpiDev epi = make_epi(epi_in);
    GemmPlan p;
    hipError_t e = plan_gemm(p, lda, C, ldc, M, N, K, epi, ws, ws_bytes, variant, splits_out != nullptr);
    if (e != hipSuccess || p.kind == GK_NONE) return e;
    const int Kp = (K + 127) / 128 * 128;
    float* partial = p.S > 1 ? ws : nullptr;
    switch (p.kind) {
        case GK_SKINNY3: e = launch_skinny3(p.p3, A, lda, Wp, C, ldc, M, N, Kp, epi, partial, st); break;
        case GK_SKINNY2: e = launch_skinny2(p.p2, A, lda, Wp, ws, M, N, K, Kp, epi.w8, epi.w8s, epi.w8_kl, st); break;
        case GK_SKINNY:
            plan_hit(PLAN_SKINNY);
            switch (p.p1.MF) {
#define SK1(MF_) launch_kernel<gemm_skinny<MF_>>(sk_class(N, K), 2.0 * (double)N * (double)K, dim3(p.p1.gx, p.S), dim3(512), p.lds, st, A, lda, Wp, ws, M, N, Kp, \
                                                 p.p1.KC, p.p1.nbpb)
                case 1: e = SK1(1); break;
                case 2: e = SK1(2); break;
                case 3: e = SK1(3); break;
                default: e = SK1(4); break;
#undef SK1
            }
            if (e == hipSuccess) e = hipGetLastError();
            break;
        default: e = launch_tiles(p, A, lda, Wp, C, ldc, M, N, K, Kp, epi, partial, variant, st); break;
    }
    if (e != hipSuccess) return e;
    if (p.done == GD_SLABS) {
        *splits_out = p.S;
        return e;
    }
    return complete_splitk(p, epi, ws, C, ldc, M, N, st);
}

hipError_t launch_gemm_skinny_partial(const bf16_t* A, int lda, const bf16_t* Wp, float* ws, size_t ws_bytes, int M, int N,
                                      int K, int* S_out, hipStream_t st, const void* w8, const float* w8s) {
    if (M <= 0 || M > 64 || N <= 0) return hipErrorInvalidValue;
    const int Kp = (K + 127) / 128 * 128;
    GemmPlan p = GemmPlan{};
    hipError_t e = plan_streaming(p, M, N, Kp, ws, ws_bytes, false, true);
    if (e != hipSuccess) return e;
    if (p.kind == GK_SKINNY3) {
        EpiDev none = make_epi(nullptr);
        if (w8 && w8s) { none.w8 = (const uint8_t*)w8; none.w8s = w8s; }
        e = launch_skinny3(p.p3, A, lda, Wp, nullptr, 0, M, N, Kp, none, ws, st);
    } else {
        e = launch_skinny2(p.p2, A, lda, Wp, ws, M, N, K, Kp, (const uint8_t*)w8, w8s, 0, st);
    }
    *S_out = p.S;
    return e;
}

__global__ __launch_bounds__(256) void quantize_rows_fp8_k(const bf16_t* __restrict__ W, int ldw, int K, float* __restrict__ scales,
                                                           bf16_t* __restrict__ Wdq) {
    __shared__ float red[16];
    const int n = blockIdx.x;
    const bf16_t* w = W + (size_t)n * ldw;
    float mx = 0.f;
    for (int k = threadIdx.x; k < K; k += blockDim.x) mx = fmaxf(mx, fabsf(bf2f(w[k])));
    mx = block_max(mx, red);
    float s = 1.0f;
    if (mx > 0.f) {
        int e;
        const float f = frexpf(mx / 448.0f, &e);
        s = ldexpf(1.0f, f == 0.5f ? e - 1 : e);
    }
    if (threadIdx.x == 0) scales[n] = s;
    const float inv = 1.0f / s;
    for (int k = threadIdx.x; k < K; k += blockDim.x) {
        const float x = bf2f(w[k]) * inv;
        const int pk = __builtin_amdgcn_cvt_pk_fp8_f32(x, 0.0f, 0, false);
        const f32x2_t back = __builtin_amdgcn_cvt_pk_f32_fp8((uint32_t)pk, false);
        Wdq[(size_t)n * ldw + k] = f2bf(back[0] * s);
    }
}

__global__ void pack_weight_fp8_k(const bf16_t* __restrict__ Wdq, int ldw, const float* __restrict__ scales, int N, int K,
                                  uint8_t* __restrict__ Wq, float* __restrict__ scales_packed, int Kp, int glu, int kl) {
    const int K64 = Kp >> 6;
    const int N16 = (N + 15) >> 4;
    const long long total = (long long)N16 * K64 * 64;
    for (long long idx = (long long)blockIdx.x * blockDim.x + threadIdx.x; idx < total; idx += (long long)gridDim.x * blockDim.x) {
        const int lane = (int)(idx & 63);
        const long long blk = idx >> 6;
        const int kb = (int)(blk % K64);
        const int nb = (int)(blk / K64);
        int n = nb * 16 + (lane & 15);
        if (glu) {
            const int half = N >> 1, i = nb >> 1;
            n = ((nb & 1) ? half : 0) + i * 16 + (lane & 15);
            if (i * 16 + (lane & 15) >= half) n = N;
        }
        const float s = n < N ? scales[n] : 1.0f, inv = 1.0f / s;
        if (kb == 0 && (lane >> 4) == 0) scales_packed[nb * 16 + (lane & 15)] = s;
        uint32_t o[4];
#pragma unroll
        for (int half_ = 0; half_ < 2; ++half_) {
            const int k = kl ? kb * 64 + (lane >> 4) * 16 + half_ * 8 : kb * 64 + half_ * 32 + (lane >> 4) * 8;
            float v[8];
#pragma unroll
            for (int e = 0; e < 8; ++e) v[e] = (n < N && k + e < K) ? bf2f(Wdq[(size_t)n * ldw + k + e]) * inv : 0.f;
            int lo = __builtin_amdgcn_cvt_pk_fp8_f32(v[0], v[1], 0, false);
            lo = __builtin_amdgcn_cvt_pk_fp8_f32(v[2], v[3], lo, true);
            int hi = __builtin_amdgcn_cvt_pk_fp8_f32(v[4], v[5], 0, false);
            hi = __builtin_amdgcn_cvt_pk_fp8_f32(v[6], v[7], hi, true);
            o[2 * half_] = (uint32_t)lo;
            o[2 * half_ + 1] = (uint32_t)hi;
        }
        *(uint4*)(Wq + idx * 16) = make_uint4(o[0], o[1], o[2], o[3]);
    }
}

hipError_t launch_quantize_rows_fp8(const bf16_t* W, int ldw, int N, int K, float* scales, bf16_t* Wdq, hipStream_t st) {
    if (N <= 0) return hipSuccess;
    hipLaunchKernelGGL(quantize_rows_fp8_k, dim3(N), dim3(256), 0, st, W, ldw, K, scales, Wdq);
    return hipGetLastError();
}
hipError_t launch_pack_weight_fp8(const bf16_t* Wdq, int ldw, const float* scales, int N, int K, uint8_t* Wq, float* scales_packed,
                                  int Kpad, int glu, hipStream_t st, int kl) {
    const long long total = (long long)((N + 15) / 16) * (Kpad / 64) * 64;
    int blocks = (int)((total + 255) / 256);
    if (blocks > 65535) blocks = 65535;
    hipLaunchKernelGGL(pack_weight_fp8_k, dim3(blocks), dim3(256), 0, st, Wdq, ldw, scales, N, K, Wq, scales_packed, Kpad, glu, kl);
    return hipGetLastError();
}

hipError_t launch_pack_weight_bf16(const bf16_t* W, int ldw, int N, int K, bf16_t* Wp, int Kpad, int glu,
                                   hipStream_t st) {
    const long long total = (long long)((N + 15) / 16) * (Kpad / 32) * 64;
    int blocks = (int)((total + 255) / 256);
// ... 5 lines not shown
```

cover_vla_amd/csrc/gemm_common.h:

```cpp
#pragma once
#include <type_traits>
#include "common.h"
#include "kernels.h"

#define BK 64
#ifndef PCTL
#define PCTL(slot) do { } while (0)
#endif

struct EpiDev {
    const float* bias;
    const void* residual;
    const float* lscale;
    int ldr, res_f32, act, glu, out_f32;
    float out_scale;
    const float* norm_w;
    const float* norm_b;
    bf16_t* norm_out;
    int ld_norm_out, norm_style;
    float norm_w_offset, norm_eps;
    const uint8_t* w8;
    const float* w8s;
    const uint8_t* a8;
    const float* a8s;
    int lda8;
    uint8_t* nq8;
    float* nq8s;
    int ldnq8;
    int w8_kl;
    const uint8_t* a8mx;
    uint8_t* o8;
    uint8_t* o8mx;
    int ldo8;
};

__device__ __forceinline__ void store_q8_chunk(uint8_t* row, int k, const float (&v)[8], float inv) {
    int lo = __builtin_amdgcn_cvt_pk_fp8_f32(v[0] * inv, v[1] * inv, 0, false);
    lo = __builtin_amdgcn_cvt_pk_fp8_f32(v[2] * inv, v[3] * inv, lo, true);
    int hi = __builtin_amdgcn_cvt_pk_fp8_f32(v[4] * inv, v[5] * inv, 0, false);
    hi = __builtin_amdgcn_cvt_pk_fp8_f32(v[6] * inv, v[7] * inv, hi, true);
    *(uint2*)(row + (k >> 6) * 64 + ((k >> 3) & 3) * 16 + ((k >> 5) & 1) * 8) = make_uint2((uint32_t)lo, (uint32_t)hi);
}
__device__ __forceinline__ float e4m3_pow2_scale(float mx) {
    float s = 1.0f;
    if (mx > 0.f) {
        int e;
        const float f = frexpf(mx / 448.0f, &e);
        s = ldexpf(1.0f, f == 0.5f ? e - 1 : e);
    }
    return s;
}
__device__ __forceinline__ uint32_t mx_quant_chunk(const float (&v)[8], uint2& q) {
    float mx = 0.f;
#pragma unroll
    for (int e = 0; e < 8; ++e) mx = fmaxf(mx, fabsf(v[e]));
    mx = fmaxf(mx, __builtin_bit_cast(float, __builtin_amdgcn_update_dpp(0, __builtin_bit_cast(int, mx), 0xB1, 0xf, 0xf, true)));
    mx = fmaxf(mx, __builtin_bit_cast(float, __builtin_amdgcn_update_dpp(0, __builtin_bit_cast(int, mx), 0x4E, 0xf, 0xf, true)));
    const float s = fmaxf(e4m3_pow2_scale(mx), 1.1754943508222875e-38f);
    const float inv = 1.0f / s;
    int lo = __builtin_amdgcn_cvt_pk_fp8_f32(v[0] * inv, v[1] * inv, 0, false);
    lo = __builtin_amdgcn_cvt_pk_fp8_f32(v[2] * inv, v[3] * inv, lo, true);
    int hi = __builtin_amdgcn_cvt_pk_fp8_f32(v[4] * inv, v[5] * inv, 0, false);
    hi = __builtin_amdgcn_cvt_pk_fp8_f32(v[6] * inv, v[7] * inv, hi, true);
    q = make_uint2((uint32_t)lo, (uint32_t)hi);
    return (__builtin_bit_cast(uint32_t, s) >> 23) & 0xffu;
}

__device__ __forceinline__ void epi_value4(const EpiDev& e, int m, int n0, int N, float v[4]) {
    const bool full = (n0 + 3 < N);
    if (full) {
        float b[4] = {0.f, 0.f, 0.f, 0.f}, ls[4] = {1.f, 1.f, 1.f, 1.f}, r[4] = {0.f, 0.f, 0.f, 0.f};
        if (e.bias) {
#pragma unroll
            for (int i = 0; i < 4; ++i) b[i] = e.bias[n0 + i];
        }
        if (e.lscale) {
#pragma unroll
            for (int i = 0; i < 4; ++i) ls[i] = e.lscale[n0 + i];
        }
        if (e.residual) {
            if (e.res_f32) {
                const float* rp = (const float*)e.residual + (size_t)m * e.ldr + n0;
#pragma unroll
                for (int i = 0; i < 4; ++i) r[i] = rp[i];
            } else {
                const bf16_t* rp = (const bf16_t*)e.residual + (size_t)m * e.ldr + n0;
#pragma unroll
                for (int i = 0; i < 4; ++i) r[i] = bf2f(rp[i]);
            }
        }
#pragma unroll
        for (int i = 0; i < 4; ++i) {
            float x = v[i];
            if (e.bias) x += b[i];
            x = bfround(x);
            if (e.act != ACT_NONE) x = bfround(act_apply_bf16(x, e.act));
            if (e.lscale) x = bfround(x * ls[i]);
            if (e.residual) x = x + r[i];
            if (e.out_scale != 1.0f) x *= e.out_scale;
            v[i] = x;
        }
        return;
    }
#pragma unroll
    for (int i = 0; i < 4; ++i) {
        float x = v[i];
        if (e.bias && (full || n0 + i < N)) x += e.bias[n0 + i];
        x = bfround(x);
        if (e.act != ACT_NONE) x = bfround(act_apply_bf16(x, e.act));
        v[i] = x;
    }
    if (e.lscale) {
#pragma unroll
        for (int i = 0; i < 4; ++i)
            if (full || n0 + i < N) v[i] = bfround(v[i] * e.lscale[n0 + i]);
    }
    if (e.residual) {
        if (e.res_f32) {
            const float* r = (const float*)e.residual + (size_t)m * e.ldr + n0;
#pragma unroll
            for (int i = 0; i < 4; ++i)
                if (full || n0 + i < N) v[i] = v[i] + r[i];
        } else {
            const bf16_t* r = (const bf16_t*)e.residual + (size_t)m * e.ldr + n0;
#pragma unroll
            for (int i = 0; i < 4; ++i)
                if (full || n0 + i < N) v[i] = v[i] + bf2f(r[i]);
        }
    }
    if (e.out_scale != 1.0f) {
#pragma unroll
        for (int i = 0; i < 4; ++i) v[i] *= e.out_scale;
    }
}
__device__ __forceinline__ bool epi_is_plain(const EpiDev& e) {
    return !e.bias && !e.residual && !e.lscale && e.act == ACT_NONE && e.out_scale == 1.0f;
}
__device__ __forceinline__ void epi_put4(const EpiDev& e, void* C, int ldc, int m, int n0, int N, const float v[4]) {
    if (n0 >= N) return;
    const bool full = (n0 + 3 < N);
    if (e.out_f32) {
        float* o = (float*)C + (size_t)m * ldc + n0;
        if (full && ((((uintptr_t)o) & 15) == 0)) {
            *(float4*)o = make_float4(v[0], v[1], v[2], v[3]);
        } else {
#pragma unroll
            for (int i = 0; i < 4; ++i)
                if (n0 + i < N) o[i] = v[i];
        }
    } else {
        bf16_t* o = (bf16_t*)C + (size_t)m * ldc + n0;
        if (full && ((((uintptr_t)o) & 7) == 0)) {
            uint2 p;
            p.x = pack_bf2(v[0], v[1]);
            p.y = pack_bf2(v[2], v[3]);
            *(uint2*)o = p;
        } else {
#pragma unroll
            for (int i = 0; i < 4; ++i)
                if (n0 + i < N) o[i] = f2bf(v[i]);
        }
    }
}

__device__ __forceinline__ void epi_store4(const EpiDev& e, void* C, int ldc, int m, int n0, int N, float v[4]) {
    if (n0 >= N) return;
    const bool full = (n0 + 3 < N);
    epi_value4(e, m, n0, N, v);
    if (e.out_f32) {
        float* o = (float*)C + (size_t)m * ldc + n0;
        if (full && ((((uintptr_t)o) & 15) == 0)) {
            *(float4*)o = make_float4(v[0], v[1], v[2], v[3]);
        } else {
            for (int i = 0; i < 4; ++i)
                if (n0 + i < N) o[i] = v[i];
        }
    } else {
        bf16_t* o = (bf16_t*)C + (size_t)m * ldc + n0;
        if (full && ((((uintptr_t)o) & 7) == 0)) {
            uint2 p;
            p.x = pack_bf2(v[0], v[1]);
            p.y = pack_bf2(v[2], v[3]);
            *(uint2*)o = p;
        } else {
            for (int i = 0; i < 4; ++i)
                if (n0 + i < N) o[i] = f2bf(v[i]);
        }
    }
}

__device__ __forceinline__ void epi_store4_glu(const EpiDev& e, void* C, int ldc, int m, int j0, int Nout, float g[4],
                                               float u[4]) {
    if (j0 >= Nout) return;
    float v[4];
#pragma unroll
    for (int i = 0; i < 4; ++i) {
        float gg = bfround(g[i]), uu = bfround(u[i]);
        gg = bfround(act_apply_bf16(gg, e.act));
        v[i] = bfround(gg * uu);
    }
    if (e.out_f32) {
        float* o = (float*)C + (size_t)m * ldc + j0;
        for (int i = 0; i < 4; ++i)
            if (j0 + i < Nout) o[i] = v[i];
    } else {
        bf16_t* o = (bf16_t*)C + (size_t)m * ldc + j0;
        if (j0 + 3 < Nout && ((((uintptr_t)o) & 7) == 0)) {
            uint2 p;
            p.x = pack_bf2(v[0], v[1]);
            p.y = pack_bf2(v[2], v[3]);
            *(uint2*)o = p;
        } else {
            for (int i = 0; i < 4; ++i)
                if (j0 + i < Nout) o[i] = f2bf(v[i]);
        }
    }
}

template <int WM, int WN, int F>
__device__ __forceinline__ void tiled_epilogue_row(f32x4 (&acc)[WN][WM], const EpiDev& epi, void* C, int ldc, int M, int N, int mw,
                                                   int nw, int r, int g, float* __restrict__ partial) {
    const int m = mw + F * 16 + r;
    if (m < M) {
        if (partial) {
#pragma unroll
            for (int b = 0; b < WN; ++b) {
                const int n = nw + b * 16 + 4 * g;
                if (n < N) {
                    float* o = partial + ((size_t)blockIdx.y * M + m) * N + n;
                    if (n + 3 < N && ((((uintptr_t)o) & 15) == 0)) {
                        *(float4*)o = make_float4(acc[b][F][0], acc[b][F][1], acc[b][F][2], acc[b][F][3]);
                    } else {
                        const float v[4] = {acc[b][F][0], acc[b][F][1], acc[b][F][2], acc[b][F][3]};
#pragma unroll
                        for (int i = 0; i < 4; ++i)
                            if (n + i < N) o[i] = v[i];
                    }
                }
            }
        } else if (epi.glu) {
#pragma unroll
            for (int b = 0; b < WN; b += 2) {
                const int nblk = (nw >> 4) + b;
                float gv[4] = {acc[b][F][0], acc[b][F][1], acc[b][F][2], acc[b][F][3]};
                float uv[4] = {acc[b + 1][F][0], acc[b + 1][F][1], acc[b + 1][F][2], acc[b + 1][F][3]};
                epi_store4_glu(epi, C, ldc, m, (nblk >> 1) * 16 + 4 * g, N >> 1, gv, uv);
            }
        } else {
            float vv[WN][4];
#pragma unroll
            for (int b = 0; b < WN; ++b) {
#pragma unroll
                for (int i = 0; i < 4; ++i) vv[b][i] = acc[b][F][i];
                const int n = nw + b * 16 + 4 * g;
                if (n < N) epi_value4(epi, m, n, N, vv[b]);
            }
#pragma unroll
            for (int b = 0; b < WN; ++b) epi_put4(epi, C, ldc, m, nw + b * 16 + 4 * g, N, vv[b]);
        }
    }
    if constexpr (F + 1 < WM) tiled_epilogue_row<WM, WN, F + 1>(acc, epi, C, ldc, M, N, mw, nw, r, g, partial);
}
template <int WM, int WN>
__device__ __forceinline__ void tiled_epilogue(f32x4 (&acc)[WN][WM], const EpiDev& epi, void* C, int ldc, int M, int N, int mw,
                                               int nw, int r, int g, float* __restrict__ partial) {
    tiled_epilogue_row<WM, WN, 0>(acc, epi, C, ldc, M, N, mw, nw, r, g, partial);
}

template <int WM, int WN, int F>
__device__ __forceinline__ void staged_fill_row(f32x4 (&acc)[WN][WM], char* st, int pitch, int m0, int n0, int mw, int nw, int r, int g,
// ... 217 lines not shown
        } else {
            if (epi.out_f32) {
                const float4 a4 = *(const float4*)(lrow + ch * 16);
                float v[4] = {a4.x, a4.y, a4.z, a4.w};
                epi_value4(epi, m, n0 + ch * 4, N, v);
                *(float4*)dst = make_float4(v[0], v[1], v[2], v[3]);
            } else {
                const float4 a4 = *(const float4*)(lrow + ch * 32), b4 = *(const float4*)(lrow + ch * 32 + 16);
                float v[4] = {a4.x, a4.y, a4.z, a4.w}, w[4] = {b4.x, b4.y, b4.z, b4.w};
                epi_value4(epi, m, n0 + ch * 8, N, v);
                epi_value4(epi, m, n0 + ch * 8 + 4, N, w);
                *(uint4*)dst = make_uint4(pack_bf2(v[0], v[1]), pack_bf2(v[2], v[3]), pack_bf2(w[0], w[1]), pack_bf2(w[2], w[3]));
            }
        }
    }
    }
}

__device__ __forceinline__ void glds16_s(uint32_t voff, const void* sbase, uint32_t lds_wave_base_u32) {
    uint32_t keep;
    asm volatile(
        "s_mov_b32 %0, m0\n\t"
        "s_mov_b32 m0, %3\n\t"
        "s_nop 0\n\t"
        "global_load_lds_dwordx4 %1, %2\n\t"
        "s_mov_b32 m0, %0"
        : "=&s"(keep)
        : "v"(voff), "s"(sbase), "s"(lds_wave_base_u32)
        : "memory");
}

__device__ __forceinline__ void glds4_s(uint32_t voff, const void* sbase, uint32_t lds_wave_base_u32) {
    uint32_t keep;
    asm volatile(
        "s_mov_b32 %0, m0\n\t"
        "s_mov_b32 m0, %3\n\t"
        "s_nop 0\n\t"
        "global_load_lds_dword %1, %2\n\t"
        "s_mov_b32 m0, %0"
        : "=&s"(keep)
        : "v"(voff), "s"(sbase), "s"(lds_wave_base_u32)
        : "memory");
}


enum TilePick {
    TP_128x128 = 0, TP_64x128 = 1, TP_64x64 = 2, TP_128x128_S4 = 3, TP_256x128 = 4, TP_128x256 = 5, TP_128x128_W8 = 6, TP_64x128_S3 = 7,
    TP_128x128_S3 = 8,
    TP_PC_64x128_S3 = 9, TP_PC_64x128 = 10, TP_PC_128x128 = 11, TP_PC_256x128 = 12, TP_PC_128x256 = 13, TP_PC_224x96_W4 = 14,
    TP_PC_224x128 = 15, TP_PC_224x192 = 16, TP_PC_224x96 = 17, TP_PC_128x192 = 18,
    PLAN_SKINNY2 = 19, PLAN_SKINNY3 = 20, PLAN_FP8 = 21, PLAN_SKINNY = 22,
    TP_V3_224x192 = 23, TP_V3_224x128 = 24, TP_V3_256x128 = 25, TP_V3_128x256 = 26, TP_V3_224x96 = 27,
    TP_V3K_224x96 = 30,
};

struct SkinnyPlan {
    int MF, KC, S, nbpb, gx;
    size_t lds, ws_bytes;
};
struct Skinny2Plan {
    int MF, KS, NBW, gx, S;
    size_t lds, ws_bytes;
};
struct Skinny3Plan {
    bool ok;
    int MF, NBW, S, kper, gx;
    size_t lds, ws_bytes;
};

enum GemmKind { GK_NONE, GK_SKINNY, GK_SKINNY2, GK_SKINNY3, GK_TILED, GK_TILED_PC, GK_F8_PC, GK_F8_V3, GK_V3 };
enum GemmDone { GD_NONE = 0, GD_REDUCE = 1, GD_REDUCE_NORM = 2, GD_SLABS = 3 };

struct GemmPlan {
    GemmKind kind;
    int slot;
    int pick;
    int S, kt_per;
    int tiles_m, tiles_n, block;
    size_t lds;
    SkinnyPlan p1;
    Skinny2Plan p2;
    Skinny3Plan p3;
    GemmDone done;
    bool norm_launch;
    int rcls;
};

template <auto kfn, typename... Args>
static inline hipError_t launch_kernel(int cls, double work, dim3 grid, dim3 block, size_t lds, hipStream_t st, Args... args) {
    if (lds > 64 * 1024) {
        static LdsAttrCache c;
        const hipError_t e = lds_attr_160k_cached((const void*)kfn, c);
        if (e != hipSuccess) return e;
    }
    hipEvent_t ea, eb;
    if (prof_enabled() && prof_reserve(cls, work, &ea, &eb) >= 0)
        hipExtLaunchKernelGGL(kfn, grid, block, (uint32_t)lds, st, ea, eb, 0, args...);
    else
        hipLaunchKernelGGL(kfn, grid, block, lds, st, args...);
    return hipSuccess;
}

bool gemm_fp8_tiled_supported(int pick);
hipError_t launch_gemm_fp8_tiled(const GemmPlan& p, const EpiDev& epi, void* C, int ldc, int M, int N, int Kp, float* partial, double prof_work,
                                 hipStream_t st);

hipError_t launch_gemm_v3(const GemmPlan& p, const bf16_t* A, int lda, const bf16_t* Wp, void* C, int ldc, int M, int N, int Kp, const EpiDev& epi,
                          float* partial, int prof_cls, double prof_work, hipStream_t st);
```

cover_vla_amd/csrc/kernels.h:

```cpp
#pragma once
#include <hip/hip_runtime.h>
#include <stdint.h>
#include "../../include/cover_hip.h"

typedef uint16_t bf16_t;

hipError_t launch_gemm_bf16(const bf16_t* A, int lda, const bf16_t* Wp, void* C, int ldc, int M, int N, int K,
                            const cover_gemm_epi* epi, float* splitk_ws, size_t splitk_ws_bytes, int variant,
                            hipStream_t st, int* splits_out = nullptr);
hipError_t launch_gemm_skinny_partial(const bf16_t* A, int lda, const bf16_t* Wp, float* ws, size_t ws_bytes, int M, int N,
                                      int K, int* S_out, hipStream_t st, const void* w8 = nullptr, const float* w8s = nullptr);
#define COVER_GEMM_PLANS 32
hipError_t gemm_plan_query(const bf16_t* A, int lda, const bf16_t* Wp, const void* C, int ldc, int M, int N, int K, const cover_gemm_epi* epi,
                           const float* ws, size_t ws_bytes, int variant, int* plan);
void gemm_plan_counts(long long* out, int n, int reset);
int gemm_v3_probe(unsigned long long* out);
hipError_t launch_quantize_rows_fp8(const bf16_t* W, int ldw, int N, int K, float* scales, bf16_t* Wdq, hipStream_t st);
hipError_t launch_pack_weight_fp8(const bf16_t* Wdq, int ldw, const float* scales, int N, int K, uint8_t* Wq, float* scales_packed,
                                  int Kpad, int glu, hipStream_t st, int kl = 0);
hipError_t launch_quantize_act_fp8(const bf16_t* X, int ldx, int M, int K, uint8_t* out, int ld8, float* scales, hipStream_t st);
hipError_t launch_quantize_act_fp8_mx(const bf16_t* X, int ldx, int M, int K, uint8_t* out, int ld8, uint8_t* mx, hipStream_t st);
hipError_t launch_pack_weight_bf16(const bf16_t* W, int ldw, int N, int K, bf16_t* Wp, int Kpad, int glu_interleave,
                                   hipStream_t st);

hipError_t launch_attention_bf16(const cover_attn_args* a, hipStream_t st);
bool attention_mx_ok(const cover_attn_args* x);
hipError_t launch_attention_bf16_pair(const cover_attn_args* a0, const cover_attn_args* a1, hipStream_t st);
hipError_t attention_plan(const cover_attn_args* a, int* plan);
hipError_t attention_pair_plan(const cover_attn_args* a0, const cover_attn_args* a1, int* dual);
hipError_t launch_decode_attention_fused(const cover_decode_attn_args* a, hipStream_t st);
hipError_t launch_decode_own_attention(const cover_own_attn_args* a, hipStream_t st);

hipError_t launch_layernorm_bf16(const bf16_t* x, int ldx, const float* w, const float* b, bf16_t* y, int ldy, int rows,
                                 int dim, float eps, hipStream_t st);
hipError_t launch_rmsnorm(const void* x, int x_f32, int ldx, const float* w, float w_offset, int style, bf16_t* y, int ldy,
                          int rows, int dim, float eps, hipStream_t st, uint8_t* q8 = nullptr, int ld8 = 0, float* q8s = nullptr);
hipError_t launch_rope_kv_write(const cover_rope_args* a, hipStream_t st);
hipError_t launch_rope_kv_write_pair(const cover_rope_args* a0, const cover_rope_args* a1, hipStream_t st);
hipError_t launch_embed_gather(const bf16_t* table, int dim, const int64_t* ids, int n, float scale, bf16_t* out,
                               int ldo, hipStream_t st);
hipError_t launch_decode_feedback(const cover_decode_feedback_args* a, hipStream_t st);
hipError_t launch_decode_feedback_lp2(const cover_decode_feedback_args* a, const float* lp2, float* lp2_out, long long ld_lp2, hipStream_t st);
hipError_t launch_decode_feedback_fsm(const cover_decode_feedback_args* a, const cover_token_fsm* f, const float* lp2, float* lp2_out,
                                      long long ld_lp2, hipStream_t st);
hipError_t launch_patchify(const cover_patchify_args* a, hipStream_t st);
hipError_t launch_copy_rows_bf16(const bf16_t* src, int lds_, bf16_t* dst, int ldd, int rows, int cols,
                                 const int* src_row_idx, const int* dst_row_idx, hipStream_t st);
hipError_t launch_add_bias_rows_bf16(bf16_t* x, int ldx, const bf16_t* add, int ld_add, int rows, int cols, int add_rows,
                                     hipStream_t st);
hipError_t launch_scale_bf16(bf16_t* x, int ldx, int rows, int cols, float pre_div, float post_mul, hipStream_t st);
hipError_t launch_cast_f32_to_bf16(const float* x, int ldx, bf16_t* y, int ldy, int rows, int cols, hipStream_t st);
hipError_t launch_cast_bf16_to_f32(const bf16_t* x, int ldx, float* y, int ldy, int rows, int cols, hipStream_t st);

hipError_t launch_gemm_f32(const cover_gemm_f32_args* a, hipStream_t st);
int gemm_f32_plan(const cover_gemm_f32_args* a, int* deep);
hipError_t launch_layernorm_f32(const float* x, int ldx, const float* w, const float* b, float* y, int ldy, int rows,
                                int dim, float eps, hipStream_t st, int rows_per_group = 0, long long wb_group_stride = 0);
hipError_t launch_softmax_rows_f32(float* x, int ldx, int rows, int cols, float scale, hipStream_t st);
hipError_t launch_l2norm_rows_f32(const float* x, int ldx, float* y, int ldy, int rows, int cols, hipStream_t st);
hipError_t launch_add_f32(const float* a, int lda, const float* b, int ldb, float* y, int ldy, int rows, int cols,
                          int b_rows, hipStream_t st);
hipError_t launch_xent_diag_f32(const float* x, int ldx, int rows, int cols, float* loss, int* rank, hipStream_t st);
hipError_t launch_act_f32(const float* x, int ldx, float* y, int ldy, int rows, int cols, int act, hipStream_t st);
hipError_t launch_mha_f32(const cover_mha_f32_args* a, hipStream_t st);
hipError_t launch_masked_mean_f32(const float* x, const uint8_t* pad, float* y, int B, int T, int D, hipStream_t st);
hipError_t launch_sincos_time_embed(const float* time, int B, int dim, double min_period, double max_period, bf16_t* out,
                                    int ldo, hipStream_t st);

hipError_t launch_token_sample(const cover_token_sample_args* a, hipStream_t st);
hipError_t launch_token_sample_scored(const cover_token_sample_scored_args* a, hipStream_t st);
hipError_t launch_token_logprob(const cover_token_logprob_args* a, hipStream_t st);
hipError_t launch_token_topn(const cover_token_topn_args* a, hipStream_t st);
hipError_t launch_token_sample_rows(const cover_token_sample_rows_args* a, hipStream_t st);
hipError_t launch_token_logprob_rows(const cover_token_logprob_rows_args* a, hipStream_t st);
hipError_t launch_token_topn_rows(const cover_token_topn_rows_args* a, hipStream_t st);
hipError_t launch_token_sample_rows_allowed(const cover_token_sample_rows_args* a, const cover_token_allow* al, hipStream_t st);
hipError_t launch_token_logprob_rows_allowed(const cover_token_logprob_rows_args* a, const cover_token_allow* al, hipStream_t st);
hipError_t launch_token_topn_rows_allowed(const cover_token_topn_rows_args* a, const cover_token_allow* al, hipStream_t st);
hipError_t launch_token_sample_rows_ref(const cover_token_sample_rows_args* a, const cover_token_allow* al ,
                                        const cover_token_ref* ref, hipStream_t st);
hipError_t launch_gumbel_topn(const cover_gumbel_topn_args* a, hipStream_t st);
hipError_t launch_token_select(const cover_token_select_args* a, hipStream_t st);
hipError_t launch_score_select(const cover_score_select_args* a, hipStream_t st);
hipError_t launch_tokens_to_histories(const int64_t* tokens, int ld_tokens, int N, int tok_vocab, const float* centers,
                                      int n_centers, const float* past, int n_past, float pad_value, float* hist, uint8_t* pad,
                                      hipStream_t st, int n_use = 1);
hipError_t launch_actions_to_histories(const float* actions, long long n_stride, long long t_stride, int N, int n_use,
                                       const float* lo_hi, const float* past, int n_past, float pad_value, float* hist,
                                       uint8_t* pad, hipStream_t st);
hipError_t launch_group_argmax(const float* scores, int N, int gs, int* result, float* best, hipStream_t st);
hipError_t launch_prior_select(const cover_prior_select_args* a, hipStream_t st);
size_t gemm_workspace_bytes(int M, int N, int K);
hipError_t launch_augment_tokens(const cover_augment_args* a, hipStream_t st);
hipError_t launch_augment_actions(const cover_augment_args* a, hipStream_t st);
hipError_t launch_proposal_prior_tokens(const cover_proposal_prior_args* a, hipStream_t st);
hipError_t launch_proposal_prior_actions(const cover_proposal_prior_args* a, hipStream_t st);
hipError_t launch_beam_merge(const cover_beam_merge_args* a, hipStream_t st);
// ... 23 lines not shown
```

cover_vla_amd/openvla.py:

```python
from __future__ import annotations

from typing import Dict, NamedTuple, Optional

import os
import weakref

import numpy as np
import torch

from . import _lib as L
from . import ops
from .graphs import ReplayGraph
from .ops import RowParam
from .models import BF, Decoder, KvGeometry, VitTower, _f32
from .sampling import PickPlan, StepOutputs

IMAGENET_MEAN, IMAGENET_STD = (0.485, 0.456, 0.406), (0.229, 0.224, 0.225)


_DecodeState = NamedTuple("_DecodeState", [(f, object) for f in ("prompt_of_cand", "cand_len", "last_row", "pos_all", "u", "prompt_slots",
                                                                  "prompt_lens", "outs", "fed")])


class OpenVLA:
    def __init__(self, sd: Dict[str, torch.Tensor], c: dict, *, device="cuda:0", max_prompts=8, max_candidates=32,
                 max_text=32, horizon=1, n_cams=1, weight_dtype="bf16", own_kv=None):
        self.c, self.dev = dict(c), torch.device(device)
        dev = self.dev
        sub = lambda p: {k[len(p):]: v for k, v in sd.items() if k.startswith(p)}
        self.n_patches = (c["image"] // c["patch"]) ** 2
        self.n_cams = n_cams
        self.dino = VitTower(sub("dino."), dim=c["dino_dim"], layers=c["dino_layers"], heads=c["dino_heads"], mlp=c["dino_mlp"],
                             patch=c["patch"], act="gelu_erf", eps=1e-6, layerscale=True, prefix_tokens=c["dino_prefix"],
                             device=device, n_layers_used=c["dino_layers"] - 1)
        self.siglip = VitTower(sub("siglip."), dim=c["sig_dim"], layers=c["sig_layers"], heads=c["sig_heads"], mlp=c["sig_mlp"],
                               patch=c["patch"], act="gelu_tanh", eps=1e-6, device=device, n_layers_used=c["sig_layers"] - 1)
        self.fused = c["dino_dim"] + c["sig_dim"]
        self.proj = [ops.pack_linear(sd[f"projector.fc{i}.weight"].to(dev), sd[f"projector.fc{i}.bias"]) for i in (1, 2, 3)]
        self.embed = sd["llm.embed_tokens.weight"].to(BF).contiguous().to(dev)
        fp8 = weight_dtype == "fp8"
        if weight_dtype not in ("bf16", "fp8"):
            raise ValueError("weight_dtype must be 'bf16' or 'fp8'")
        self.weight_dtype = weight_dtype
        if own_kv not in (None, "bf16", "fp8"):
            raise ValueError("own_kv must be None, 'bf16' or 'fp8'")
        self.own_kv = own_kv
        self.lm_head = ops.pack_linear(sd["lm_head.weight"].to(dev), fp8=fp8)
        lo, hi = c["tok_vocab"] - c["n_bins"], c["tok_vocab"]
        self.lm_head_actions = ops.pack_linear(sd["lm_head.weight"][lo:hi].to(dev), fp8=fp8)
        self.n_gen = 7 * horizon
        self.T0 = 1 + self.n_patches * n_cams
        geom = KvGeometry(c["Hkv"], c["D"], [1, max_prompts, max_candidates], [self.T0, max_text, self.n_gen])
        self.llm = Decoder(sub("llm."), dim=c["llm_dim"], layers=c["llm_layers"], Hq=c["Hq"], Hkv=c["Hkv"], D=c["D"],
                           mlp=c["llm_mlp"], act="silu", norm="llama", eps=1e-5, rope="hf", n_pos=self.T0 + max_text + self.n_gen + 8,
                           device=device, cache=geom, fp8_weights=fp8)
        self.max_prompts, self.max_candidates, self.max_text = max_prompts, max_candidates, max_text
        self.llm.reserve(self.T0 + max_prompts * max_text)
        D = c["llm_dim"]
        self.action_lo = c["tok_vocab"] - c["n_bins"]
        self.action_hi = c["tok_vocab"]
        self.x_pre = torch.empty(self.T0 + max_prompts * max_text, D, dtype=BF, device=dev)
        self.x_dec = torch.empty(max_candidates, D, dtype=BF, device=dev)
        self.h_sel = torch.empty(max_candidates, D, dtype=BF, device=dev)
        self.logits = torch.empty(max_candidates, c["vocab"], dtype=torch.float32, device=dev)
        self.head_ws = ops.gemm_workspace(max_candidates, c["vocab"], D, dev)
        self.logits_actions = torch.empty(max_candidates, c["n_bins"], dtype=torch.float32, device=dev)
        self.head_ws_actions = ops.gemm_workspace(max_candidates, c["n_bins"], D, dev)
        self.hn = torch.empty(max_candidates, D, dtype=BF, device=dev)
        self.kept_sel = torch.empty(max_candidates, dtype=torch.int32, device=dev)
        self.zero_slots = torch.zeros(max(max_prompts, max_candidates), dtype=torch.int32, device=dev)
        self.bos = torch.tensor([1], dtype=torch.int64, device=dev)
        self._side = None
        self._weak = weakref.proxy(self)
        self._vis = {}
        self._bos_ready = False
        self.vision_graph = os.environ.get("COVER_VISION_GRAPH", "1") != "0"
        self.slice_action_head = os.environ.get("COVER_ACTION_HEAD", "0") == "1"
        self.vision_overlap = True
        self.decode_graph = os.environ.get("COVER_DECODE_GRAPH", "1") != "0"
        self._dec = {}

    def _ensure_bos_kv(self):
        if self._bos_ready:
            return
        x = ops.embed_gather(self.embed, self.bos)
        pos = torch.zeros(1, dtype=torch.int32, device=self.dev)
        g = self.llm.group(1, 1, pos, [dict(region=0, length=1, mask=ops.MASK_CAUSAL)], 0)
        self.llm.forward(x, [g], final_norm=False)
        self._bos_ready = True

    def _vision_static(self, n, H, W):
        key = (n, H, W)
        st = self._vis.get(key)
        if st is None:
            c, P, dev = self.c, self.n_patches, self.dev
            bufs = dict(frame=torch.empty(n, H, W, 3, dtype=torch.uint8, device=dev),
                        d=self.dino.static_bufs(n, H, W), s=self.siglip.static_bufs(n, H, W),
                        fused=torch.empty(n * P, self.fused, dtype=BF, device=dev),
                        h=[torch.empty(n * P, lin.n_out, dtype=BF, device=dev) for lin in self.proj],
                        ws=[ops.gemm_workspace(n * P, lin.N, lin.K, dev) for lin in self.proj])
            me, dino, siglip = self._weak, self.dino, self.siglip
            st = self._vis[key] = dict(bufs, graph=ReplayGraph(lambda: me._encode_static(bufs), dev, gen=lambda: (dino.ws_gen, siglip.ws_gen)))
        return st

    def _encode_static(self, st) -> torch.Tensor:
        c = self.c
        n, P = st["frame"].shape[0], self.n_patches
        mul_d = [1.0 / (255.0 * s) for s in IMAGENET_STD]
        add_d = [-m / s for m, s in zip(IMAGENET_MEAN, IMAGENET_STD)]
        main = torch.cuda.current_stream()
        if self._side is None:
            self._side = torch.cuda.Stream(device=self.dev)
        side = self._side if self.vision_overlap else main
        side.wait_stream(main)
        with torch.cuda.stream(side):
            xs = self.siglip.embed(st["frame"], [1.0 / (255.0 * 0.5)] * 3, [-1.0] * 3, bufs=st["s"])
            xs = self.siglip.forward(xs)
        xd = self.dino.embed(st["frame"], mul_d, add_d, bufs=st["d"])
        xd = self.dino.forward(xd)
        main.wait_stream(side)
        fused = st["fused"].view(n, P, self.fused)
        fused[:, :, :c["dino_dim"]].copy_(xd[:, c["dino_prefix"]:, :])
        fused[:, :, c["dino_dim"]:].copy_(xs)
        h = ops.gemm(st["fused"], self.proj[0], act="gelu_erf", out=st["h"][0], ws=st["ws"][0])
        h = ops.gemm(h, self.proj[1], act="gelu_erf", out=st["h"][1], ws=st["ws"][1])
        return ops.gemm(h, self.proj[2], out=st["h"][2], ws=st["ws"][2])

    def encode_image(self, frame_u8: torch.Tensor) -> torch.Tensor:
        n, H, W, _ = frame_u8.shape
        st = self._vision_static(n, H, W)
        st["frame"].copy_(frame_u8)
        if not self.vision_graph:
            return self._encode_static(st)
        st["graph"].run()
        return st["h"][2]

    def _prefill(self, frame_u8, prompt_tokens, mark=lambda name: None, on_vision_enqueued=None, on_prefill_enqueued=None):
        dev = self.dev
        P, Lt = prompt_tokens.shape
        T0 = self.T0
        Tp = T0 - 1
        self._ensure_bos_kv()
        x = self.x_pre[: Tp + P * Lt]
        mark("start")
        x[:Tp].copy_(self.encode_image(frame_u8))
        if on_vision_enqueued is not None:
            on_vision_enqueued()
        mark("vision")
        ops.embed_gather(self.embed, prompt_tokens.reshape(-1).contiguous(), out=x[Tp:])
        pos0 = 1 + torch.arange(Tp, dtype=torch.int32, device=dev)
        pos1 = (T0 + torch.arange(Lt, dtype=torch.int32, device=dev))[None].expand(P, Lt).contiguous()
        g0 = self.llm.group(1, Tp, pos0, [dict(region=0, length=T0, mask=ops.MASK_CAUSAL, causal_offset=1)], 0, write_t_off=1)
        g1 = self.llm.group(P, Lt, pos1.view(-1),
                            [dict(region=0, length=T0, slot_of_batch=self.zero_slots),
                             dict(region=1, length=Lt, mask=ops.MASK_CAUSAL)], 1)
        self.llm.forward(x, [g0, g1], final_norm=False)
        mark("prefill")
        if on_prefill_enqueued is not None:
            on_prefill_enqueued()
        return x

    def _cand_rows(self, prompt_lens, P, Lt, per_prompt):
        dev, T0 = self.dev, self.T0
        N = P * per_prompt
        prompt_of_cand = (torch.arange(N, device=dev) // per_prompt).to(torch.int32)
        cand_len = prompt_lens.to(torch.int32)[prompt_of_cand.long()].contiguous()
        last_row = (T0 - 1 + prompt_of_cand * Lt + cand_len - 1).to(torch.int32)
        pos_all = ((T0 + cand_len)[None, :] + torch.arange(self.n_gen, dtype=torch.int32, device=dev)[:, None]).contiguous()
        return prompt_of_cand, cand_len, last_row, pos_all

    def sample(self, frame_u8: torch.Tensor, prompt_tokens: torch.Tensor, prompt_lens: torch.Tensor, n_samples: int,
               uniforms: Optional[torch.Tensor] = None, temperature: RowParam = 1.0, trace: Optional[dict] = None,
               force_tokens: Optional[torch.Tensor] = None, on_prefill_enqueued=None, on_vision_enqueued=None,
               top_k: RowParam = 0, top_p: RowParam = 1.0, return_logprobs: bool = False, top_logprobs: int = 0,
               prior_temperature: Optional[float] = None):
        dev = self.dev
        P, Lt = prompt_tokens.shape
        N = P * n_samples
        plan = PickPlan.resolve("sample", "candidate", N, dev, has_uniforms=uniforms is not None, params=(temperature, top_k, top_p),
                                top_logprobs=top_logprobs, prior_temperature=prior_temperature, filter_always=False)

        def mark(name):
            if trace is not None and "events" in trace:
                ev = torch.cuda.Event(enable_timing=True)
                ev.record()
                trace["events"].append((name, ev))

        if P > self.max_prompts or N > self.max_candidates or Lt > self.max_text:
            raise ValueError("prompts/candidates/text length exceed the sizes this model was built for")
        x = self._prefill(frame_u8, prompt_tokens, mark, on_vision_enqueued, on_prefill_enqueued)
        prompt_of_cand, cand_len, last_row, pos_all = self._cand_rows(prompt_lens, P, Lt, n_samples)
        u_t = None if uniforms is None else uniforms.to(torch.float32).t().contiguous()
        new_outs = lambda: StepOutputs.alloc(self.n_gen, N, dev, logit=True, logprob=return_logprobs, ref=plan.t_ref is not None, n_top=plan.n_top, fill=None)
        if self.decode_graph and trace is None and force_tokens is None and not self.slice_action_head:
            key = (P, n_samples, Lt) + plan.graph_key(return_logprobs)
            st = self._dec.get(key)
            if st is None:
                outs = new_outs()
                st_plan = plan._replace(rp=None if plan.rp is None else tuple(torch.empty_like(t) for t in plan.rp))
                st_state = _DecodeState(prompt_of_cand.clone(), torch.empty_like(cand_len), torch.empty_like(last_row), torch.empty_like(pos_all),
                                        None if u_t is None else torch.empty_like(u_t), torch.arange(P, dtype=torch.int32, device=dev),
                                        torch.empty(P, dtype=torch.int32, device=dev), outs, outs.tokens)
                me, llm = self._weak, self.llm
                st = self._dec[key] = dict(graph=ReplayGraph(lambda: me._decode_body(x, st_plan, st_state), dev, gen=lambda: llm.ws_gen), plan=st_plan, state=st_state)
            s = st["state"]
            s.cand_len.copy_(cand_len); s.last_row.copy_(last_row); s.pos_all.copy_(pos_all)
            s.prompt_lens.copy_(prompt_lens.to(torch.int32))
            if u_t is not None:
                s.u.copy_(u_t)
            for dst, src in zip(st["plan"].rp or (), plan.rp or ()):
                dst.copy_(src)
            st["graph"].run()
            return s.outs.result()
        outs = new_outs()
        state = _DecodeState(prompt_of_cand, cand_len, last_row, pos_all, u_t, torch.arange(P, dtype=torch.int32, device=dev),
                             prompt_lens.to(torch.int32).contiguous(), outs, outs.tokens if force_tokens is None else force_tokens.t().contiguous())
        self._decode_body(x, plan, state, trace, mark)
        return outs.result()

    def _decode_body(self, x, plan, s, trace=None, mark=lambda name: None):
        D, T0 = self.c["llm_dim"], self.T0
        N, P = s.cand_len.shape[0], s.prompt_slots.shape[0]
        Lt = (x.shape[0] - (T0 - 1)) // P
        ops.copy_rows(x, self.h_sel, N, D, s.last_row, None)
        self._head_pick(self.h_sel[:N], 0, plan, s, trace)
        xd = self.x_dec[:N]
        own = {}
        if self.own_kv is not None:
            own = dict(own_kv=self.own_kv, seg1_group=N // P, seg1_slot_of_group=s.prompt_slots, seg1_len_of_group=s.prompt_lens)
        for i in range(1, self.n_gen):
            ops.embed_gather(self.embed, s.fed[i - 1], out=xd)
            g = self.llm.group(N, 1, s.pos_all[i - 1],
                               [dict(region=0, length=T0, slot_of_batch=self.zero_slots),
                                dict(region=1, length=Lt, len_of_batch=s.cand_len, slot_of_batch=s.prompt_of_cand),
                                dict(region=2, length=i)], 2, write_t_off=i - 1, seg0_shared=True, **own)
            self.llm.forward(xd, [g], final_norm=False)
            self._head_pick(xd, i, plan, s, trace)
            mark(f"decode{i}")

    def _head_pick(self, h, i, plan, s, trace):
        N, o = h.shape[0], s.outs
        u = None if s.u is None else s.u[i]
        out = dict(out_logit=o.sel[i], out_kept=self.kept_sel[:N], out_logprob=None if o.lps is None else o.lps[i],
                   out_ref=None if o.prior is None else o.prior[i], top=o.top_at(i))
        hn = self._final_norm(h)
        if not plan.greedy and (trace is None or "events" in trace) and self.slice_action_head:
            lg = ops.gemm(hn, self.lm_head_actions, out=self.logits_actions[:N], ws=self.head_ws_actions)
            t, _, _ = plan.pick(lg, 0, self.c["n_bins"], u, **out)
            torch.add(t, self.action_lo, out=o.tokens[i])
            if o.top is not None:
                o.top[0][i].add_((o.top[0][i] >= 0) * self.action_lo)
            return
        lg = self._full_head(hn, trace)
        lo, hi = (0, self.c["tok_vocab"]) if plan.greedy else (self.action_lo, self.action_hi)
        plan.pick(lg, lo, hi, u, out_tok=o.tokens[i], **out)

    def _final_norm(self, h):
        return ops.rmsnorm(h, self.llm.final_norm, 1e-5, w_offset=0.0, style=1, out=self.hn[:h.shape[0]])

    def _full_head(self, hn, trace):
        lg = ops.gemm(hn, self.lm_head, out=self.logits[:hn.shape[0]], ws=self.head_ws)
        if trace is not None and "events" not in trace:
            trace.setdefault("logits", []).append(lg.clone())
        return lg

    def beam_search(self, frame_u8: torch.Tensor, prompt_tokens: torch.Tensor, prompt_lens: torch.Tensor, n_beams: int, *,
                    trace: Optional[dict] = None):
        return self._beam_loop("beam_search", frame_u8, prompt_tokens, prompt_lens, n_beams, trace)[:3]

    def stochastic_beam_search(self, frame_u8: torch.Tensor, prompt_tokens: torch.Tensor, prompt_lens: torch.Tensor, n_beams: int,
                               uniforms: torch.Tensor, temperature: float = 1.0, *, trace: Optional[dict] = None):
        return self._beam_loop("stochastic_beam_search", frame_u8, prompt_tokens, prompt_lens, n_beams, trace, uniforms, temperature)

    def _beam_loop(self, what, frame_u8, prompt_tokens, prompt_lens, n_beams, trace, uniforms=None, temperature=1.0):
        dev = self.dev
        P, Lt = prompt_tokens.shape
        B = int(n_beams)
        if not 1 <= B <= 64:
            raise ValueError(f"{what}: 1 <= n_beams <= 64 is required (got {n_beams})")
        N = P * B
        if self.own_kv is not None:
            raise ValueError(f"{what}: the head-major own-token cache (own_kv) is not supported; build the model with own_kv=None")
        if 2 * N > self.max_candidates:
            raise ValueError(f"{what}: the own-token K/V ping-pong between two sets of N = {N} slots: build the model with "
                             f"max_candidates >= {2 * N} (twice the candidates; it has {self.max_candidates})")
        if P > self.max_prompts or Lt > self.max_text:
            raise ValueError("prompts/text length exceed the sizes this model was built for")
        S, T0, lo, hi = self.n_gen, self.T0, self.action_lo, self.action_hi
        keyed = uniforms is not None
        if keyed:
            if not temperature > 0:
                raise ValueError(f"{what}: temperature > 0 is required (got {temperature})")
            if uniforms.dtype != torch.float32 or tuple(uniforms.shape) != (S, N, hi - lo) or uniforms.device != torch.device(dev):
                raise ValueError(f"{what}: uniforms must be fp32 [n_gen, N, n_bins] = [{S}, {N}, {hi - lo}] on {dev} "
                                 f"(got {uniforms.dtype} {tuple(uniforms.shape)} on {uniforms.device})")
            uniforms = uniforms.contiguous()
        x = self._prefill(frame_u8, prompt_tokens)
        prompt_of_cand, cand_len, last_row, pos_all = self._cand_rows(prompt_lens, P, Lt, B)
        i32, f32 = dict(dtype=torch.int32, device=dev), dict(dtype=torch.float32, device=dev)
        parent = torch.empty(S, N, **i32)
        token, feed = torch.empty(S, N, dtype=torch.int64, device=dev), torch.empty(S, N, dtype=torch.int64, device=dev)
        step_lp = torch.empty(S, N, **f32)
        cum = torch.full((S + 1, N), float("-inf"), **f32)
        cum[0, ::B] = 0.0
        cand_tok, cand_lp = torch.empty(N, B, dtype=torch.int64, device=dev), torch.empty(N, B, **f32)
        ent = torch.empty(N, **f32)
        if keyed:
            pert = torch.full((S + 1, N), float("-inf"), **f32)
            pert[0, ::B] = 0.0
            cand_g, kappa = torch.empty(N, B, **f32), torch.empty(P, **f32)
        rows = torch.arange(N, **i32)
        slots = (rows, rows + N)
        src_base = tuple(s - s % B for s in (rows + N, rows))
        src, dead = torch.empty(N, **i32), torch.empty(N, dtype=torch.bool, device=dev)
        k_tab, vt_tab = self.llm.kv_tables()
        region = self.llm.kv_region(2)
        out_tokens, out_lps = torch.empty(N, S, dtype=torch.int64, device=dev), torch.empty(N, S, **f32)
        xd = self.x_dec[:N]

        def head_merge(h, i):
            lg = self._full_head(self._final_norm(h), trace)
            outs = dict(out_parent=parent[i], out_token=token[i], out_feed=feed[i], out_cum=cum[i + 1], out_step_lp=step_lp[i])
            if keyed:
                ops.gumbel_topn(lg, lo, hi, B, cum[i], pert[i], uniforms[i], temperature, out_tok=cand_tok, out_logprob=cand_lp,
                                out_perturbed=cand_g)
                ops.beam_merge_gumbel(cum[i], cand_tok, cand_lp, cand_g, B, lo, out_g=pert[i + 1], out_kappa=kappa, **outs)
            else:
                ops.token_topn(lg, lo, hi, B, 1.0, 0, 1.0, out_tok=cand_tok, out_logprob=cand_lp, out_entropy=ent)
                ops.beam_merge(cum[i], cand_tok, cand_lp, B, lo, **outs)
            if trace is not None:
                step = dict(parent=parent[i].clone(), token=token[i].clone(), cum=cum[i + 1].clone(),
                            cand_tok=cand_tok.clone(), cand_lp=cand_lp.clone())
                if keyed:
                    step.update(cand_g=cand_g.clone(), g=pert[i + 1].clone(), kappa=kappa.clone())
                trace.setdefault("beam", []).append(step)

        ops.copy_rows(x, self.h_sel, N, self.c["llm_dim"], last_row, None)
        head_merge(self.h_sel[:N], 0)
        for i in range(1, S):
            h = i & 1
            ops.embed_gather(self.embed, feed[i - 1], out=xd)
            torch.lt(parent[i - 1], 0, out=dead)
            torch.add(src_base[h], parent[i - 1], out=src)
# ... 32 lines not shown
```

cover_vla_amd/ops.py:

```python
from __future__ import annotations

import ctypes as C
import math
from dataclasses import dataclass
from typing import NamedTuple, Optional, Sequence, Union

import numpy as np
import torch

from . import _lib as L
from .graphs import Graph, PooledGraph, Timer, _stream

ACT = {"none": 0, "gelu_tanh": 1, "gelu_erf": 2, "silu": 3, "relu": 4}
MASK_LEN, MASK_CAUSAL, MASK_VISLEN = 0, 1, 2


def _ptr(t: Optional[torch.Tensor]) -> Optional[int]:
    return None if t is None else t.data_ptr()


def _chk_dev(*ts):
    for t in ts:
        if t is not None and not t.is_cuda:
            raise L.CoverError("cover_vla_amd ops need device tensors: there is no CPU path")
# ... 1 lines not shown

@dataclass
class PackedLinear:
    wp: torch.Tensor
    N: int
    K: int
    bias: Optional[torch.Tensor] = None
    glu: bool = False
    w8: Optional[torch.Tensor] = None
    w8s: Optional[torch.Tensor] = None
    use_w8: bool = True
    klinear: bool = False

    @property
    def n_out(self) -> int:
        return self.N // 2 if self.glu else self.N

    @property
    def kp(self) -> int:
        return (self.K + 127) // 128 * 128


def pack_linear(weight: torch.Tensor, bias: Optional[torch.Tensor] = None, glu: bool = False, fp8: bool = False,
                klinear: bool = False) -> PackedLinear:
    assert not (klinear and (glu or not fp8))
    _chk_dev(weight)
    w = weight.to(torch.bfloat16).contiguous()
    N, K = w.shape
    h = L.lib()
    w8 = w8s = None
    if fp8:
        scales = torch.empty(N, dtype=torch.float32, device=w.device)
        wdq = torch.empty_like(w)
        L.check(h.cover_quantize_rows_fp8(w.data_ptr(), K, N, K, scales.data_ptr(), wdq.data_ptr(), _stream()), "quantize_rows_fp8")
        w8 = torch.empty(h.cover_packed_weight_fp8_bytes(N, K), dtype=torch.uint8, device=w.device)
        w8s = torch.empty((N + 15) // 16 * 16, dtype=torch.float32, device=w.device)
        if klinear:
            L.check(h.cover_pack_weight_fp8_klinear(wdq.data_ptr(), K, scales.data_ptr(), N, K, w8.data_ptr(), w8s.data_ptr(), _stream()),
                    "pack_weight_fp8_klinear")
        else:
            L.check(h.cover_pack_weight_fp8(wdq.data_ptr(), K, scales.data_ptr(), N, K, w8.data_ptr(), w8s.data_ptr(), 1 if glu else 0,
                                            _stream()), "pack_weight_fp8")
        w = wdq
    nbytes = h.cover_packed_weight_bytes(N, K)
    wp = torch.empty(nbytes // 2, dtype=torch.bfloat16, device=w.device)
    L.check(h.cover_pack_weight_bf16(w.data_ptr(), K, N, K, wp.data_ptr(), 1 if glu else 0, _stream()), "pack_weight")
    b = None if bias is None else bias.detach().to(torch.bfloat16).to(torch.float32).contiguous().to(w.device)
    return PackedLinear(wp, N, K, b, glu, w8, w8s, klinear=klinear)


def quantize_act_fp8(x: torch.Tensor, K: Optional[int] = None):
    _chk_dev(x)
    assert x.dtype == torch.bfloat16 and x.dim() == 2 and x.stride(1) == 1
    M = x.shape[0]
    K = x.shape[1] if K is None else K
    kp = (K + 127) // 128 * 128
    q = torch.empty(M, kp, dtype=torch.uint8, device=x.device)
    sc = torch.empty(M, dtype=torch.float32, device=x.device)
    L.check(L.lib().cover_quantize_act_fp8(x.data_ptr(), x.stride(0), M, K, q.data_ptr(), kp, sc.data_ptr(), _stream()), "quantize_act_fp8")
    return q, sc


def quantize_act_fp8_mx(x: torch.Tensor, K: Optional[int] = None):
    _chk_dev(x)
    assert x.dtype == torch.bfloat16 and x.dim() == 2 and x.stride(1) == 1
    M = x.shape[0]
    K = x.shape[1] if K is None else K
    kp = (K + 127) // 128 * 128
    q = torch.empty(M, kp, dtype=torch.uint8, device=x.device)
    mx = torch.empty(kp // 128, M, 4, dtype=torch.uint8, device=x.device)
    L.check(L.lib().cover_quantize_act_fp8_mx(x.data_ptr(), x.stride(0), M, K, q.data_ptr(), kp, mx.data_ptr(), _stream()), "quantize_act_fp8_mx")
    return q, mx


def gemm_workspace(M: int, N: int, K: int, device) -> Optional[torch.Tensor]:
    n = L.lib().cover_gemm_workspace_bytes(M, N, K)
    return torch.empty(max(n, 4) // 4, dtype=torch.float32, device=device) if n else None


def gemm(a: torch.Tensor, lin: PackedLinear, *, act: str = "none", residual: Optional[torch.Tensor] = None,
         layer_scale: Optional[torch.Tensor] = None, out: Optional[torch.Tensor] = None, out_f32: bool = False,
         out_scale: float = 1.0, variant: int = 0, ws: Optional[torch.Tensor] = None, norm_w: Optional[torch.Tensor] = None,
         norm_out: Optional[torch.Tensor] = None, norm_style: int = 0, norm_w_offset: float = 0.0, norm_eps: float = 1e-6,
         norm_b: Optional[torch.Tensor] = None, a8: Optional[tuple] = None, out8: Optional[tuple] = None) -> torch.Tensor:
    _chk_dev(a, residual, out)
    assert a.dtype == torch.bfloat16 and a.dim() == 2 and a.stride(1) == 1
    M = a.shape[0]
    h = L.lib()
    if out is None:
        out = torch.empty(M, lin.n_out, dtype=torch.float32 if out_f32 else torch.bfloat16, device=a.device)
    e = L.GemmEpi()
    e.bias = _ptr(lin.bias)
    e.residual = _ptr(residual)
    e.ld_residual = residual.stride(0) if residual is not None else 0
    e.residual_f32 = 1 if (residual is not None and residual.dtype == torch.float32) else 0
    e.layer_scale = _ptr(layer_scale)
    e.act = ACT[act]
    e.glu = 1 if lin.glu else 0
    e.out_f32 = 1 if out.dtype == torch.float32 else 0
    e.out_scale = out_scale
    if lin.w8 is not None and lin.use_w8:
        e.w8, e.w8_scale = lin.w8.data_ptr(), lin.w8s.data_ptr()
        e.w8_klinear = 1 if lin.klinear else 0
        if a8 is not None:
            q, qs = a8
            _chk_dev(q, qs)
            assert q.dtype == torch.uint8 and q.shape[0] == M and q.stride(1) == 1
            if lin.klinear:
                assert qs.dtype == torch.uint8 and qs.is_contiguous() and tuple(qs.shape) == (lin.kp // 128, M, 4)
                e.a8, e.a8_mx, e.ld_a8 = q.data_ptr(), qs.data_ptr(), q.stride(0)
            else:
                assert qs.dtype == torch.float32
                e.a8, e.a8_scale, e.ld_a8 = q.data_ptr(), qs.data_ptr(), q.stride(0)
    if out8 is not None:
        q, qs = out8
        _chk_dev(q, qs)
        assert q.dtype == torch.uint8 and q.shape[0] == M and q.stride(1) == 1 and qs.dtype == torch.uint8 and qs.is_contiguous()
        assert tuple(qs.shape) == ((lin.n_out + 127) // 128, M, 4)
        e.out8, e.out8_mx, e.ld_out8 = q.data_ptr(), qs.data_ptr(), q.stride(0)
    if norm_w is not None:
        e.norm_w, e.norm_out, e.ld_norm_out = norm_w.data_ptr(), norm_out.data_ptr(), norm_out.stride(0)
        e.norm_style, e.norm_w_offset, e.norm_eps = norm_style, norm_w_offset, norm_eps
        e.norm_b = _ptr(norm_b)
    if ws is None:
        ws = gemm_workspace(M, lin.N, lin.K, a.device)
    L.check(h.cover_gemm_bf16(a.data_ptr(), a.stride(0), lin.wp.data_ptr(), out.data_ptr(), out.stride(0), M, lin.N,
                              lin.K, C.byref(e), _ptr(ws), ws.numel() * 4 if ws is not None else 0, variant,
                              _stream()), "gemm_bf16")
    return out


def gemm_probe() -> dict:
    torch.cuda.synchronize()
    buf = (C.c_ulonglong * 16)()
    L.check(L.lib().cover_gemm_probe(buf), "gemm_probe")
    w0, w1, w2, w3, c0, c1, nk = (int(buf[i]) for i in range(7))
    e4, e5, e6 = (int(buf[i]) for i in (12, 13, 14))
    loop_us = (w2 - w1) * 0.01
    staged = w2 <= e4 <= e5 <= e6 <= w3
    return dict(prologue_us=(w1 - w0) * 0.01, loop_us=loop_us, epilogue_us=(w3 - w2) * 0.01, k_tiles=nk,
                cycles_per_k_tile=(c1 - c0) / max(nk, 1), clock_ghz=(c1 - c0) / max(loop_us, 1e-9) / 1e3,
                epilogue_split_us=[(e4 - w2) * 0.01, (e5 - e4) * 0.01, (e6 - e5) * 0.01, (w3 - e6) * 0.01] if staged else None)


def gemm_plan_counts(reset: bool = False) -> list:
    n = 32
    buf = (C.c_longlong * n)()
    L.lib().cover_gemm_plan_counts(buf, n, 1 if reset else 0)
    return list(buf)


@dataclass
class Segment:
    k: torch.Tensor
    vt: torch.Tensor
    k_strides: Sequence[int]
    vt_strides: Sequence[int]
    length: int = 0
    len_of_batch: Optional[torch.Tensor] = None
    slot_of_batch: Optional[torch.Tensor] = None
    mask: int = MASK_LEN
    causal_offset: int = 0
    vis_len: Optional[torch.Tensor] = None
    k_offset: int = 0
    vt_offset: int = 0


def fill_segment(s: L.KvSegment, seg: Segment) -> None:
    s.k = seg.k.data_ptr() + 2 * seg.k_offset
    s.vt = seg.vt.data_ptr() + 2 * seg.vt_offset
    s.k_slot_stride, s.k_t_stride, s.k_h_stride = seg.k_strides
    s.vt_slot_stride, s.vt_h_stride, s.vt_d_stride = seg.vt_strides
    s.slot_of_batch = _ptr(seg.slot_of_batch)
    s.len_of_batch = _ptr(seg.len_of_batch)
    s.vis_len = _ptr(seg.vis_len)
    s.len = seg.length
    s.mask_mode = seg.mask
    s.causal_offset = seg.causal_offset


def attention_args(q: torch.Tensor, q_strides: Sequence[int], out: Optional[torch.Tensor], o_strides: Sequence[int], B: int, Tq: int,
                   Hq: int, Hkv: int, D: int, scale: float, segments: Sequence[Segment], state_in=None, state_out=None, out8=None) -> "L.AttnArgs":
    _chk_dev(q, out)
    a = L.AttnArgs()
    a._keep = (q, out, out8, state_in, state_out, list(segments))
    a.q, a.out = q.data_ptr(), _ptr(out)
    if out8 is not None:
        _chk_dev(out8[0], out8[1])
        assert out8[0].dtype == torch.uint8 and out8[1].dtype == torch.uint8 and out8[1].is_contiguous() and out8[0].is_contiguous()
        a.out8, a.out8_mx, a.out8_rows = out8[0].data_ptr(), out8[1].data_ptr(), out8[0].shape[0]
    if state_in is not None:
        a.state_in_o, a.state_in_ml = state_in[0].data_ptr(), state_in[1].data_ptr()
    if state_out is not None:
        a.state_out_o, a.state_out_ml = state_out[0].data_ptr(), state_out[1].data_ptr()
    a.q_b_stride, a.q_t_stride, a.q_h_stride = q_strides
    a.o_b_stride, a.o_t_stride, a.o_h_stride = o_strides
    a.B, a.Tq, a.Hq, a.Hkv, a.D, a.scale = B, Tq, Hq, Hkv, D, scale
    a.n_seg = len(segments)
    for i, sg in enumerate(segments[:3]):
        fill_segment(a.seg[i], sg)
    return a


def attention(q: torch.Tensor, q_strides: Sequence[int], out: Optional[torch.Tensor], o_strides: Sequence[int], B: int, Tq: int,
              Hq: int, Hkv: int, D: int, scale: float, segments: Sequence[Segment], state_in=None, state_out=None, out8=None):
    a = attention_args(q, q_strides, out, o_strides, B, Tq, Hq, Hkv, D, scale, segments, state_in, state_out, out8)
    L.check(L.lib().cover_attention_bf16(C.byref(a), _stream()), "attention_bf16")
    return out


ATTN_FORMS = {-1: None, 0: "PER_TILE", 1: "KSPLIT4", 2: "KSPLIT8", 3: "SHARED"}

# ... 1193 lines not shown
```

include/cover_hip.h:

```cpp
#ifndef COVER_HIP_H
#define COVER_HIP_H
#include <stddef.h>
#include <stdint.h>

#ifdef __cplusplus
extern "C" {
#endif

#define COVER_ABI_VERSION 1

enum cover_status { COVER_OK = 0, COVER_EINVAL = -1, COVER_EHIP = -2, COVER_EWORKSPACE = -3, COVER_EUNSUPPORTED = -4 };
enum cover_act { COVER_ACT_NONE = 0, COVER_ACT_GELU_TANH = 1, COVER_ACT_GELU_ERF = 2, COVER_ACT_SILU = 3, COVER_ACT_RELU = 4 };

int cover_abi_version(void);
const char* cover_last_error(void);
int cover_device_info(int dev, int* n_cu, size_t* total_mem, char* name, int name_len);

typedef struct cover_gemm_epi {
    const float* bias;
    const void* residual;
    const float* layer_scale;
    int ld_residual;
    int residual_f32;
    int act;
    int glu;
    int out_f32;
    float out_scale;
    const float* norm_w;
    void* norm_out;
    int ld_norm_out;
    int norm_style;
    float norm_w_offset;
    float norm_eps;
    const float* norm_b;
    const void* w8;
    const float* w8_scale;
    const void* a8;
    const float* a8_scale;
    int ld_a8;
    int ld_norm_out8;
    void* norm_out8;
    float* norm_out8_scale;
    const void* a8_mx;
    void* out8;
    void* out8_mx;
    int ld_out8;
    int w8_klinear;
} cover_gemm_epi;

size_t cover_packed_weight_bytes(int N, int K);
int cover_packed_k(int K);
int cover_pack_weight_bf16(const void* W, int ldw, int N, int K, void* Wp, int glu_interleave, void* stream);

size_t cover_packed_weight_fp8_bytes(int N, int K);
int cover_quantize_rows_fp8(const void* W, int ldw, int N, int K, float* scales, void* Wdq, void* stream);
int cover_pack_weight_fp8(const void* Wdq, int ldw, const float* scales, int N, int K, void* Wq, float* scales_packed,
                          int glu_interleave, void* stream);

int cover_quantize_act_fp8(const void* X, int ldx, int M, int K, void* out8, int ld8, float* scales, void* stream);
int cover_quantize_act_fp8_mx(const void* X, int ldx, int M, int K, void* out8, int ld8, void* mx, void* stream);
int cover_pack_weight_fp8_klinear(const void* Wdq, int ldw, const float* scales, int N, int K, void* Wq, float* scales_packed, void* stream);

size_t cover_gemm_workspace_bytes(int M, int N, int K);
int cover_gemm_bf16(const void* A, int lda, const void* Wp, void* C, int ldc, int M, int N, int K,
                    const cover_gemm_epi* epi, void* splitk_ws, size_t splitk_ws_bytes, int variant, void* stream);
int cover_gemm_plan_counts(long long* counts, int n, int reset);
int cover_gemm_plan(const void* A, int lda, const void* Wp, void* C, int ldc, int M, int N, int K,
                    const cover_gemm_epi* epi, void* splitk_ws, size_t splitk_ws_bytes, int variant, int plan[6]);
int cover_gemm_probe(unsigned long long* out);

enum cover_mask_mode { COVER_MASK_LEN = 0, COVER_MASK_CAUSAL = 1, COVER_MASK_VISLEN = 2 };
typedef struct cover_kv_segment {
    const void* k;
    const void* vt;
    long long k_slot_stride, k_t_stride, k_h_stride;
    long long vt_slot_stride, vt_h_stride, vt_d_stride;
    const int* slot_of_batch;
    const int* len_of_batch;
    const int* vis_len;
    int len;
    int mask_mode;
    int causal_offset;
    int _pad;
} cover_kv_segment;

typedef struct cover_attn_args {
    const void* q;
    void* out;
    long long q_b_stride, q_t_stride, q_h_stride;
    long long o_b_stride, o_t_stride, o_h_stride;
    int B, Tq, Hq, Hkv, D;
    float scale;
    int n_seg;
    int _pad;
    cover_kv_segment seg[3];
    const float* state_in_o; const float* state_in_ml;
    float* state_out_o; float* state_out_ml;
    void* out8; void* out8_mx;
    int out8_rows; int _pad2;
} cover_attn_args;
int cover_attention_bf16(const cover_attn_args* args, void* stream);
int cover_attention_plan(const cover_attn_args* args, int plan[4]);
int cover_attention_bf16_pair(const cover_attn_args* a0, const cover_attn_args* a1, void* stream);
int cover_attention_pair_plan(const cover_attn_args* a0, const cover_attn_args* a1, int* dual);

typedef struct cover_decode_attn_args {
    const void* qkv; int ld_qkv;
    int n_splits;
    const float* partial; const float* bias;
    int N, H, D;
    float scale;
    const int* positions; const float* cos_table; const float* sin_table; int n_pos; int rope_mode;
    cover_kv_segment seg[3];
    int write_t; int _pad;
    void* out; long long out_row_stride;
} cover_decode_attn_args;
int cover_decode_attention_fused(const cover_decode_attn_args* args, void* stream);

typedef struct cover_own_attn_args {
    void* qkv; int ld_qkv;
    int N, H, D;
    float scale;
    const int* positions; const float* cos_table; const float* sin_table; int n_pos; int rope_mode;
    void* k; void* v;
    float* k_scale; float* v_scale;
    int fp8; int t_cap;
    long long slot_stride;
    const int* slot_of_batch;
    int write_t; int _pad;
    float* state_o; float* state_ml;
} cover_own_attn_args;
int cover_decode_own_attention(const cover_own_attn_args* args, void* stream);

int cover_layernorm_bf16(const void* x, int ldx, const float* w, const float* b, void* y, int ldy, int rows, int dim,
                         float eps, void* stream);
int cover_rmsnorm_bf16(const void* x, int x_f32, int ldx, const float* w, float w_offset, int style, void* y, int ldy,
                       int rows, int dim, float eps, void* stream);
int cover_rmsnorm_bf16_q8(const void* x, int x_f32, int ldx, const float* w, float w_offset, int style, void* y, int ldy,
                          int rows, int dim, float eps, void* q8, int ld8, float* q8s, void* stream);

typedef struct cover_rope_args {
    void* qkv; int ld_qkv;
    int B, T, Hq, Hkv, D;
    const int* positions;
    const float* cos_table; const float* sin_table; int n_pos;
    int rope_mode;
    void* k_cache;
    long long k_slot_stride, k_t_stride, k_h_stride;
    void* vt_cache;
    long long vt_slot_stride, vt_h_stride, vt_d_stride;
    const int* slot_of_batch;
// ... 425 lines not shown
```

Baseline: 960.1 candidates/s.

## Compute only action-token columns of LM head via windowed skinny GEMM launch

Adds a column window (n_begin/n_end) to the GEMM epilogue. The skinny GEMM kernels launch only the block columns covering that window, and the split-K reduce and stores are restricted to it. In sampling mode the decode step now runs the LM head over just the 256 action-bin rows of the full packed weight, instead of the whole vocabulary, and this path is on by default. The change also lets the sliced head path be captured in the decode graph. It depends on the window offset mapping being correct and leaves the non-action logits unwritten.

```diff
diff --git a/cover_vla_amd/_lib.py b/cover_vla_amd/_lib.py
--- a/cover_vla_amd/_lib.py
+++ b/cover_vla_amd/_lib.py
@@ -24,7 +24,7 @@
                 ("norm_w", c_p), ("norm_out", c_p), ("ld_norm_out", c_i), ("norm_style", c_i), ("norm_w_offset", c_f),
                 ("norm_eps", c_f), ("norm_b", c_p), ("w8", c_p), ("w8_scale", c_p), ("a8", c_p), ("a8_scale", c_p), ("ld_a8", c_i), ("ld_norm_out8", c_i),
                 ("norm_out8", c_p), ("norm_out8_scale", c_p),
-                ("a8_mx", c_p), ("out8", c_p), ("out8_mx", c_p), ("ld_out8", c_i), ("w8_klinear", c_i)]
+                ("a8_mx", c_p), ("out8", c_p), ("out8_mx", c_p), ("ld_out8", c_i), ("w8_klinear", c_i), ("n_begin", c_i), ("n_end", c_i)]
 
 
 class KvSegment(C.Structure):
@@ -297,6 +297,7 @@
     "cover_gemm_bf16": (c_i, [c_p, c_i, c_p, c_p, c_i, c_i, c_i, c_i, _P(GemmEpi), c_p, C.c_size_t, c_i, c_p]),
     "cover_gemm_plan_counts": (c_i, [C.POINTER(C.c_longlong), c_i, c_i]),
     "cover_gemm_plan": (c_i, [c_p, c_i, c_p, c_p, c_i, c_i, c_i, c_i, _P(GemmEpi), c_p, C.c_size_t, c_i, C.POINTER(c_i)]),
+    "cover_gemm_plan_grid": (c_i, [c_p, c_i, c_p, c_p, c_i, c_i, c_i, c_i, _P(GemmEpi), c_p, C.c_size_t, c_i, C.POINTER(c_i), C.POINTER(c_i)]),
     "cover_gemm_probe": (c_i, [C.POINTER(C.c_ulonglong)]),
     "cover_attention_bf16": (c_i, [_P(AttnArgs), c_p]),
     "cover_attention_plan": (c_i, [_P(AttnArgs), _P(c_i)]),
diff --git a/cover_vla_amd/csrc/capi.hip b/cover_vla_amd/csrc/capi.hip
--- a/cover_vla_amd/csrc/capi.hip
+++ b/cover_vla_amd/csrc/capi.hip
@@ -98,6 +98,13 @@
     if (!plan) return fail(COVER_EINVAL, "cover_gemm_plan: null plan");
     if (const char* why = gemm_args_error(A, lda, Wp, C, N, K, epi)) return fail(COVER_EINVAL, why);
     HIPCHK(gemm_plan_query((const bf16_t*)A, lda, (const bf16_t*)Wp, C, ldc, M, N, K, epi, (const float*)ws, ws_bytes, variant, plan), "gemm_plan");
+    return COVER_OK;
+}
+int cover_gemm_plan_grid(const void* A, int lda, const void* Wp, void* C, int ldc, int M, int N, int K,
+                         const cover_gemm_epi* epi, void* ws, size_t ws_bytes, int variant, int plan[6], int grid[6]) {
+    if (!plan || !grid) return fail(COVER_EINVAL, "cover_gemm_plan_grid: null plan");
+    if (const char* why = gemm_args_error(A, lda, Wp, C, N, K, epi)) return fail(COVER_EINVAL, why);
+    HIPCHK(gemm_plan_query((const bf16_t*)A, lda, (const bf16_t*)Wp, C, ldc, M, N, K, epi, (const float*)ws, ws_bytes, variant, plan, grid), "gemm_plan_grid");
     return COVER_OK;
 }
 int cover_gemm_bf16(const void* A, int lda, const void* Wp, void* C, int ldc, int M, int N, int K,
diff --git a/cover_vla_amd/csrc/gemm_bf16.hip b/cover_vla_amd/csrc/gemm_bf16.hip
--- a/cover_vla_amd/csrc/gemm_bf16.hip
+++ b/cover_vla_amd/csrc/gemm_bf16.hip
@@ -673,7 +673,7 @@
 
 template <int MF, int KS, int NBW, bool W8 = false>
 __global__ __launch_bounds__(512) void gemm_skinny2(const bf16_t* __restrict__ A, int lda, const bf16_t* __restrict__ Wp,
-                                                    float* __restrict__ partial, int M, int N, int Kp, const float* __restrict__ wscale, int kl) {
+                                                    float* __restrict__ partial, int M, int N, int Kp, const float* __restrict__ wscale, int kl, int bx0) {
     constexpr int NG = 8 / KS, KC = 256 * KS, NBPB = NG * NBW;
     extern __shared__ __attribute__((aligned(16))) char smem[];
     const int tid = threadIdx.x, lane = tid & 63;
@@ -684,7 +684,7 @@
     const int kc = min(KC, Kp - k0);
     const int K32 = Kp >> 5;
     const int N16 = (N + 15) >> 4;
-    const int nb_begin = blockIdx.x * NBPB;
+    const int nb_begin = (blockIdx.x + bx0) * NBPB;
     const int kw0 = ks * 256;
     const int nsteps = max(0, min(8, (kc - kw0) >> 5));
     f32x4 acc[NBW][MF];
@@ -849,7 +849,7 @@
 template <int MF, int KS, int NBW, int NBUF, bool W8 = false>
 __global__ __launch_bounds__(512) void gemm_skinny3(const bf16_t* __restrict__ A, int lda, const bf16_t* __restrict__ Wp,
                                                     void* C, int ldc, int M, int N, int Kp, EpiDev epi,
-                                                    float* __restrict__ partial, int kper, const float* __restrict__ wscale, int kl) {
+                                                    float* __restrict__ partial, int kper, const float* __restrict__ wscale, int kl, int bx0) {
     SKT(0);
     constexpr int NG = 8 / KS, KC = 256 * KS, NBPB = NG * NBW;
     constexpr int XB = MF * 16 * KC * 2;
@@ -860,7 +860,7 @@
     const int ks = w % KS, ng = w / KS;
     const int K32 = Kp >> 5;
     const int N16 = (N + 15) >> 4;
-    const int nb_begin = blockIdx.x * NBPB;
+    const int nb_begin = (blockIdx.x + bx0) * NBPB;
     const int kb = blockIdx.y * kper;
     const int ke = min(Kp, kb + kper);
     const int nchunks = (ke - kb + KC - 1) / KC;
@@ -1101,7 +1101,8 @@
                 if (nb < N16 && m < M) {
                     float v[4];
                     slice_sum(gsel, ii, f, v);
-                    epi_store4(epi, C, ldc, m, nb * 16 + 4 * g, N, v);
+                    if (epi.n1 > 0) epi_store4_win(epi, C, ldc, m, nb * 16 + 4 * g, N, v);
+                    else epi_store4(epi, C, ldc, m, nb * 16 + 4 * g, N, v);
                 }
             }
         }
@@ -1112,12 +1113,14 @@
 __global__ __launch_bounds__(256) void splitk_reduce(const float* __restrict__ partial, int S, void* C, int ldc, int M,
                                                      int N, EpiDev epi) {
     const int Nout = epi.glu ? (N >> 1) : N;
-    const int groups = (Nout + 3) >> 2;
+    const bool win = epi.n1 > 0;
+    const int c0 = win ? (epi.n0 & ~3) : 0;
+    const int groups = ((win ? min(epi.n1, Nout) : Nout) - c0 + 3) >> 2;
     const long long total = (long long)M * groups;
     for (long long idx = (long long)blockIdx.x * blockDim.x + threadIdx.x; idx < total;
          idx += (long long)gridDim.x * blockDim.x) {
         const int m = (int)(idx / groups);
-        const int j0 = (int)(idx - (long long)m * groups) * 4;
+        const int j0 = c0 + (int)(idx - (long long)m * groups) * 4;
         if (epi.glu) {
             const int ng = (j0 >> 4) * 32 + (j0 & 15);
             float gv[4] = {0, 0, 0, 0}, uv[4] = {0, 0, 0, 0};
@@ -1156,7 +1159,8 @@
                         if (j0 + i < N) v[i] += p[i];
                 }
             }
-            epi_store4(epi, C, ldc, m, j0, N, v);
+            if (win) epi_store4_win(epi, C, ldc, m, j0, N, v);
+            else epi_store4(epi, C, ldc, m, j0, N, v);
         }
     }
 }
@@ -1225,6 +1229,8 @@
     d.o8mx = e ? (uint8_t*)e->out8_mx : nullptr;
     d.ldo8 = e ? e->ld_out8 : 0;
     if (!d.o8 || !d.o8mx) { d.o8 = nullptr; d.o8mx = nullptr; }
+    d.n0 = e ? e->n_begin : 0;
+    d.n1 = e ? e->n_end : 0;
     return d;
 }
 
@@ -1530,6 +1536,16 @@
         e = hipSuccess;
     } else e = plan_tiles(p, lda, M, N, Kp, epi, ws, ws_bytes, variant, mx_any);
     if (e != hipSuccess) return e;
+    if (p.kind == GK_SKINNY2) p.gx = p.p2.gx;
+    else if (p.kind == GK_SKINNY3) p.gx = p.p3.gx;
+    p.bx0 = 0; p.nbx = p.gx;
+    if (epi.n0 != 0 || epi.n1 != 0) {
+        if (epi.n0 < 0 || epi.n1 <= epi.n0 || epi.n1 > N || epi.glu || epi.norm_out || mx_any) return hipErrorInvalidValue;
+        if (p.kind != GK_SKINNY2 && p.kind != GK_SKINNY3) return hipErrorInvalidValue;
+        const int nbpb = p.kind == GK_SKINNY3 ? 2 * p.p3.NBW : (8 / p.p2.KS) * p.p2.NBW;
+        p.bx0 = (epi.n0 >> 4) / nbpb;
+        p.nbx = ((epi.n1 - 1) >> 4) / nbpb - p.bx0 + 1;
+    }
     const bool want_norm = epi.norm_w != nullptr && epi.norm_out != nullptr;
     const bool streaming = p.kind == GK_SKINNY || p.kind == GK_SKINNY2 || p.kind == GK_SKINNY3;
     const bool split = streaming ? !(p.kind == GK_SKINNY3 && p.S == 1) : p.S > 1;
@@ -1545,12 +1561,17 @@
 }
 
 hipError_t gemm_plan_query(const bf16_t* A, int lda, const bf16_t* Wp, const void* C, int ldc, int M, int N, int K, const cover_gemm_epi* epi_in,
-                           const float* ws, size_t ws_bytes, int variant, int* plan) {
+                           const float* ws, size_t ws_bytes, int variant, int* plan, int* grid) {
     GemmPlan p;
     const hipError_t e = plan_gemm(p, lda, C, ldc, M, N, K, make_epi(epi_in), ws, ws_bytes, variant, false);
     if (e != hipSuccess) return e;
     const int out[6] = {p.slot, p.pick, p.kind == GK_F8_V3 ? 1 : 0, p.S, p.done == GD_NONE ? 0 : p.done == GD_REDUCE ? 1 : 2, p.norm_launch ? 1 : 0};
     for (int i = 0; i < 6; ++i) plan[i] = out[i];
+    if (grid) {
+        const bool s2 = p.kind == GK_SKINNY2, s3 = p.kind == GK_SKINNY3;
+        const int g[6] = {s3 ? p.p3.NBW : s2 ? p.p2.NBW : 0, s3 ? 4 : s2 ? p.p2.KS : 0, s3 ? p.p3.kper : s2 ? 256 * p.p2.KS : 0, p.gx, p.bx0, p.nbx};
+        for (int i = 0; i < 6; ++i) grid[i] = g[i];
+    }
     return hipSuccess;
 }
 
@@ -1567,7 +1588,7 @@
         e = launch_kernel<splitk_reduce_norm>(p.rcls, 0.0, dim3(M), dim3(512), 0, st, ws, p.S, (bf16_t*)C, ldc, M, N, epi);
     } else if (p.done == GD_REDUCE) {
         const int Nout = epi.glu ? N / 2 : N;
-        const long long total = (long long)M * ((Nout + 3) / 4);
+        const long long total = (long long)M * ((epi.n1 > 0 ? epi.n1 - (epi.n0 & ~3) + 3 : Nout + 3) / 4);
         int rb = (int)((total + 255) / 256);
         if (rb > 2048) rb = 2048;
         e = launch_kernel<splitk_reduce>(p.rcls, 0.0, dim3(rb), dim3(256), 0, st, ws, p.S, C, ldc, M, N, epi);
@@ -1578,11 +1599,12 @@
 }
 
 static hipError_t launch_skinny2(const Skinny2Plan& p, const bf16_t* A, int lda, const bf16_t* Wp, float* ws, int M, int N, int K, int Kp,
-                                 const uint8_t* w8, const float* w8s, int kl, hipStream_t st) {
-    const dim3 grid(p.gx, p.S), block(512);
+                                 const uint8_t* w8, const float* w8s, int kl, int bx0, int nbx, hipStream_t st) {
+    const dim3 grid(nbx, p.S), block(512);
+    const int Ns = nbx < p.gx ? min(N, nbx * (8 / p.KS) * p.NBW * 16) : N;
     plan_hit(PLAN_SKINNY2);
-#define SK2(MF_, KS_, NBW_, W8_) launch_kernel<gemm_skinny2<MF_, KS_, NBW_, W8_>>(sk_class(N, K), (W8_ ? 1.0 : 2.0) * (double)N * (double)K, grid, block, p.lds, st, \
-                                                                                   A, lda, W8_ ? (const bf16_t*)w8 : Wp, ws, M, N, Kp, w8s, kl)
+#define SK2(MF_, KS_, NBW_, W8_) launch_kernel<gemm_skinny2<MF_, KS_, NBW_, W8_>>(sk_class(Ns, K), (W8_ ? 1.0 : 2.0) * (double)Ns * (double)K, grid, block, p.lds, st, \
+                                                                                   A, lda, W8_ ? (const bf16_t*)w8 : Wp, ws, M, N, Kp, w8s, kl, bx0)
     hipError_t e;
     if (w8 && w8s && p.MF <= 2) {
         if (p.MF == 1) e = p.NBW == 6 ? SK2(1, 4, 6, true) : p.NBW == 4 ? SK2(1, 4, 4, true) : p.NBW == 3 ? SK2(1, 4, 3, true) : SK2(1, 4, 2, true);
@@ -1599,11 +1621,12 @@
 }
 
 static hipError_t launch_skinny3(const Skinny3Plan& p, const bf16_t* A, int lda, const bf16_t* Wp, void* C, int ldc, int M, int N,
-                                 int Kp, const EpiDev& epi, float* partial, hipStream_t st) {
-    const dim3 grid(p.gx, p.S), block(512);
+                                 int Kp, const EpiDev& epi, float* partial, int bx0, int nbx, hipStream_t st) {
+    const dim3 grid(nbx, p.S), block(512);
+    const int Ns = nbx < p.gx ? min(N, nbx * 2 * p.NBW * 16) : N;
     plan_hit(PLAN_SKINNY3);
-#define SK3(MF_, NBW_, W8_) launch_kernel<gemm_skinny3<MF_, 4, NBW_, NBW_, W8_>>(sk_class(N, Kp), (W8_ ? 1.0 : 2.0) * (double)N * (double)Kp, grid, block, p.lds, st, \
-                                                                                  A, lda, W8_ ? (const bf16_t*)epi.w8 : Wp, C, ldc, M, N, Kp, epi, partial, p.kper, epi.w8s, epi.w8_kl)
+#define SK3(MF_, NBW_, W8_) launch_kernel<gemm_skinny3<MF_, 4, NBW_, NBW_, W8_>>(sk_class(Ns, Kp), (W8_ ? 1.0 : 2.0) * (double)Ns * (double)Kp, grid, block, p.lds, st, \
+                                                                                  A, lda, W8_ ? (const bf16_t*)epi.w8 : Wp, C, ldc, M, N, Kp, epi, partial, p.kper, epi.w8s, epi.w8_kl, bx0)
     hipError_t e;
     if (epi.w8) {
         if (p.MF == 1) e = p.NBW == 4 ? SK3(1, 4, true) : p.NBW == 3 ? SK3(1, 3, true) : SK3(1, 2, true);
@@ -1664,8 +1687,8 @@
     const int Kp = (K + 127) / 128 * 128;
     float* partial = p.S > 1 ? ws : nullptr;
     switch (p.kind) {
-        case GK_SKINNY3: e = launch_skinny3(p.p3, A, lda, Wp, C, ldc, M, N, Kp, epi, partial, st); break;
-        case GK_SKINNY2: e = launch_skinny2(p.p2, A, lda, Wp, ws, M, N, K, Kp, epi.w8, epi.w8s, epi.w8_kl, st); break;
+        case GK_SKINNY3: e = launch_skinny3(p.p3, A, lda, Wp, C, ldc, M, N, Kp, epi, partial, p.bx0, p.nbx, st); break;
+        case GK_SKINNY2: e = launch_skinny2(p.p2, A, lda, Wp, ws, M, N, K, Kp, epi.w8, epi.w8s, epi.w8_kl, p.bx0, p.nbx, st); break;
         case GK_SKINNY:
             plan_hit(PLAN_SKINNY);
             switch (p.p1.MF) {
@@ -1699,9 +1722,9 @@
     if (p.kind == GK_SKINNY3) {
         EpiDev none = make_epi(nullptr);
         if (w8 && w8s) { none.w8 = (const uint8_t*)w8; none.w8s = w8s; }
-        e = launch_skinny3(p.p3, A, lda, Wp, nullptr, 0, M, N, Kp, none, ws, st);
+        e = launch_skinny3(p.p3, A, lda, Wp, nullptr, 0, M, N, Kp, none, ws, 0, p.p3.gx, st);
     } else {
-        e = launch_skinny2(p.p2, A, lda, Wp, ws, M, N, K, Kp, (const uint8_t*)w8, w8s, 0, st);
+        e = launch_skinny2(p.p2, A, lda, Wp, ws, M, N, K, Kp, (const uint8_t*)w8, w8s, 0, 0, p.p2.gx, st);
     }
     *S_out = p.S;
     return e;
diff --git a/cover_vla_amd/csrc/gemm_common.h b/cover_vla_amd/csrc/gemm_common.h
--- a/cover_vla_amd/csrc/gemm_common.h
+++ b/cover_vla_amd/csrc/gemm_common.h
@@ -32,6 +32,7 @@
     uint8_t* o8;
     uint8_t* o8mx;
     int ldo8;
+    int n0, n1;
 };
 
 __device__ __forceinline__ void store_q8_chunk(uint8_t* row, int k, const float (&v)[8], float inv) {
@@ -186,6 +187,19 @@
             for (int i = 0; i < 4; ++i)
                 if (n0 + i < N) o[i] = f2bf(v[i]);
         }
+    }
+}
+
+__device__ __forceinline__ void epi_store4_win(const EpiDev& e, void* C, int ldc, int m, int n0, int N, float v[4]) {
+    const int hi = min(e.n1, N);
+    if (n0 >= hi || n0 + 3 < e.n0) return;
+    epi_value4(e, m, n0, N, v);
+#pragma unroll
+    for (int i = 0; i < 4; ++i) {
+        const int n = n0 + i;
+        if (n < e.n0 || n >= hi) continue;
+        if (e.out_f32) ((float*)C)[(size_t)m * ldc + (n - e.n0)] = v[i];
+        else ((bf16_t*)C)[(size_t)m * ldc + (n - e.n0)] = f2bf(v[i]);
     }
 }
 
@@ -569,6 +583,7 @@
     Skinny2Plan p2;
     Skinny3Plan p3;
     GemmDone done;
+    int gx, bx0, nbx;
     bool norm_launch;
     int rcls;
 };
diff --git a/cover_vla_amd/csrc/kernels.h b/cover_vla_amd/csrc/kernels.h
--- a/cover_vla_amd/csrc/kernels.h
+++ b/cover_vla_amd/csrc/kernels.h
@@ -12,7 +12,7 @@
                                       int K, int* S_out, hipStream_t st, const void* w8 = nullptr, const float* w8s = nullptr);
 #define COVER_GEMM_PLANS 32
 hipError_t gemm_plan_query(const bf16_t* A, int lda, const bf16_t* Wp, const void* C, int ldc, int M, int N, int K, const cover_gemm_epi* epi,
-                           const float* ws, size_t ws_bytes, int variant, int* plan);
+                           const float* ws, size_t ws_bytes, int variant, int* plan, int* grid = nullptr);
 void gemm_plan_counts(long long* out, int n, int reset);
 int gemm_v3_probe(unsigned long long* out);
 hipError_t launch_quantize_rows_fp8(const bf16_t* W, int ldw, int N, int K, float* scales, bf16_t* Wdq, hipStream_t st);
diff --git a/cover_vla_amd/openvla.py b/cover_vla_amd/openvla.py
--- a/cover_vla_amd/openvla.py
+++ b/cover_vla_amd/openvla.py
@@ -46,8 +46,6 @@
             raise ValueError("own_kv must be None, 'bf16' or 'fp8'")
         self.own_kv = own_kv
         self.lm_head = ops.pack_linear(sd["lm_head.weight"].to(dev), fp8=fp8)
-        lo, hi = c["tok_vocab"] - c["n_bins"], c["tok_vocab"]
-        self.lm_head_actions = ops.pack_linear(sd["lm_head.weight"][lo:hi].to(dev), fp8=fp8)
         self.n_gen = 7 * horizon
         self.T0 = 1 + self.n_patches * n_cams
         geom = KvGeometry(c["Hkv"], c["D"], [1, max_prompts, max_candidates], [self.T0, max_text, self.n_gen])
@@ -64,8 +62,7 @@
         self.h_sel = torch.empty(max_candidates, D, dtype=BF, device=dev)
         self.logits = torch.empty(max_candidates, c["vocab"], dtype=torch.float32, device=dev)
         self.head_ws = ops.gemm_workspace(max_candidates, c["vocab"], D, dev)
-        self.logits_actions = torch.empty(max_candidates, c["n_bins"], dtype=torch.float32, device=dev)
-        self.head_ws_actions = ops.gemm_workspace(max_candidates, c["n_bins"], D, dev)
+        self.logits_actions = self.logits[:, self.action_lo:self.action_hi]
         self.hn = torch.empty(max_candidates, D, dtype=BF, device=dev)
         self.kept_sel = torch.empty(max_candidates, dtype=torch.int32, device=dev)
         self.zero_slots = torch.zeros(max(max_prompts, max_candidates), dtype=torch.int32, device=dev)
@@ -75,7 +72,8 @@
         self._vis = {}
         self._bos_ready = False
         self.vision_graph = os.environ.get("COVER_VISION_GRAPH", "1") != "0"
-        self.slice_action_head = os.environ.get("COVER_ACTION_HEAD", "0") == "1"
+        self.slice_action_head = os.environ.get("COVER_ACTION_HEAD", "1") != "0"
+        self.head_launches = {"window": 0, "full": 0}
         self.vision_overlap = True
         self.decode_graph = os.environ.get("COVER_DECODE_GRAPH", "1") != "0"
         self._dec = {}
@@ -192,8 +190,8 @@
         prompt_of_cand, cand_len, last_row, pos_all = self._cand_rows(prompt_lens, P, Lt, n_samples)
         u_t = None if uniforms is None else uniforms.to(torch.float32).t().contiguous()
         new_outs = lambda: StepOutputs.alloc(self.n_gen, N, dev, logit=True, logprob=return_logprobs, ref=plan.t_ref is not None, n_top=plan.n_top, fill=None)
-        if self.decode_graph and trace is None and force_tokens is None and not self.slice_action_head:
-            key = (P, n_samples, Lt) + plan.graph_key(return_logprobs)
+        if self.decode_graph and trace is None and force_tokens is None:
+            key = (P, n_samples, Lt, bool(self.slice_action_head)) + plan.graph_key(return_logprobs)
             st = self._dec.get(key)
             if st is None:
                 outs = new_outs()
@@ -244,21 +242,20 @@
         out = dict(out_logit=o.sel[i], out_kept=self.kept_sel[:N], out_logprob=None if o.lps is None else o.lps[i],
                    out_ref=None if o.prior is None else o.prior[i], top=o.top_at(i))
         hn = self._final_norm(h)
-        if not plan.greedy and (trace is None or "events" in trace) and self.slice_action_head:
-            lg = ops.gemm(hn, self.lm_head_actions, out=self.logits_actions[:N], ws=self.head_ws_actions)
-            t, _, _ = plan.pick(lg, 0, self.c["n_bins"], u, **out)
-            torch.add(t, self.action_lo, out=o.tokens[i])
-            if o.top is not None:
-                o.top[0][i].add_((o.top[0][i] >= 0) * self.action_lo)
-            return
-        lg = self._full_head(hn, trace)
         lo, hi = (0, self.c["tok_vocab"]) if plan.greedy else (self.action_lo, self.action_hi)
+        if not plan.greedy and (trace is None or "events" in trace) and self.slice_action_head and N <= 64:
+            self.head_launches["window"] += 1
+            ops.gemm(hn, self.lm_head, out=self.logits_actions[:N], ws=self.head_ws, window=(lo, hi))
+            lg = self.logits[:N]
+        else:
+            lg = self._full_head(hn, trace)
         plan.pick(lg, lo, hi, u, out_tok=o.tokens[i], **out)
 
     def _final_norm(self, h):
         return ops.rmsnorm(h, self.llm.final_norm, 1e-5, w_offset=0.0, style=1, out=self.hn[:h.shape[0]])
 
     def _full_head(self, hn, trace):
+        self.head_launches["full"] += 1
         lg = ops.gemm(hn, self.lm_head, out=self.logits[:hn.shape[0]], ws=self.head_ws)
         if trace is not None and "events" not in trace:
             trace.setdefault("logits", []).append(lg.clone())
diff --git a/cover_vla_amd/ops.py b/cover_vla_amd/ops.py
--- a/cover_vla_amd/ops.py
+++ b/cover_vla_amd/ops.py
@@ -107,14 +107,18 @@
          layer_scale: Optional[torch.Tensor] = None, out: Optional[torch.Tensor] = None, out_f32: bool = False,
          out_scale: float = 1.0, variant: int = 0, ws: Optional[torch.Tensor] = None, norm_w: Optional[torch.Tensor] = None,
          norm_out: Optional[torch.Tensor] = None, norm_style: int = 0, norm_w_offset: float = 0.0, norm_eps: float = 1e-6,
-         norm_b: Optional[torch.Tensor] = None, a8: Optional[tuple] = None, out8: Optional[tuple] = None) -> torch.Tensor:
+         norm_b: Optional[torch.Tensor] = None, a8: Optional[tuple] = None, out8: Optional[tuple] = None,
+         window: Optional[tuple] = None) -> torch.Tensor:
     _chk_dev(a, residual, out)
     assert a.dtype == torch.bfloat16 and a.dim() == 2 and a.stride(1) == 1
     M = a.shape[0]
     h = L.lib()
     if out is None:
-        out = torch.empty(M, lin.n_out, dtype=torch.float32 if out_f32 else torch.bfloat16, device=a.device)
+        out = torch.empty(M, lin.n_out if window is None else window[1] - window[0], dtype=torch.float32 if out_f32 else torch.bfloat16, device=a.device)
     e = L.GemmEpi()
+    if window is not None:
+        e.n_begin, e.n_end = int(window[0]), int(window[1])
+        assert 0 <= e.n_begin < e.n_end <= lin.N and out.shape[1] >= e.n_end - e.n_begin, "gemm: bad column window"
     e.bias = _ptr(lin.bias)
     e.residual = _ptr(residual)
     e.ld_residual = residual.stride(0) if residual is not None else 0
@@ -153,6 +157,23 @@
                               lin.K, C.byref(e), _ptr(ws), ws.numel() * 4 if ws is not None else 0, variant,
                               _stream()), "gemm_bf16")
     return out
+
+
+def gemm_plan_grid(M: int, N: int, K: int, *, window: Optional[tuple] = None, out_f32: bool = False, variant: int = 0,
+                   ws_bytes: Optional[int] = None):
+    h = L.lib()
+    e = L.GemmEpi()
+    e.out_scale, e.out_f32 = 1.0, 1 if out_f32 else 0
+    if window is not None:
+        e.n_begin, e.n_end = int(window[0]), int(window[1])
+    if ws_bytes is None:
+        ws_bytes = h.cover_gemm_workspace_bytes(M, N, K)
+    plan, grid = (C.c_int * 6)(), (C.c_int * 6)()
+    fake = 0x10000000
+    kp = (K + 127) // 128 * 128
+    rc = h.cover_gemm_plan_grid(fake, kp, 2 * fake, 3 * fake, N if window is None else window[1] - window[0], M, N, K, C.byref(e),
+                                4 * fake if ws_bytes else None, ws_bytes, variant, plan, grid)
+    return (tuple(plan), tuple(grid)) if rc == 0 else None
 
 
 def gemm_probe() -> dict:
diff --git a/include/cover_hip.h b/include/cover_hip.h
--- a/include/cover_hip.h
+++ b/include/cover_hip.h
@@ -46,6 +46,7 @@
     void* out8_mx;
     int ld_out8;
     int w8_klinear;
+    int n_begin, n_end;
 } cover_gemm_epi;
 
 size_t cover_packed_weight_bytes(int N, int K);
@@ -67,6 +68,8 @@
 int cover_gemm_plan_counts(long long* counts, int n, int reset);
 int cover_gemm_plan(const void* A, int lda, const void* Wp, void* C, int ldc, int M, int N, int K,
                     const cover_gemm_epi* epi, void* splitk_ws, size_t splitk_ws_bytes, int variant, int plan[6]);
+int cover_gemm_plan_grid(const void* A, int lda, const void* Wp, void* C, int ldc, int M, int N, int K,
+                         const cover_gemm_epi* epi, void* splitk_ws, size_t splitk_ws_bytes, int variant, int plan[6], int grid[6]);
 int cover_gemm_probe(unsigned long long* out);
 
 enum cover_mask_mode { COVER_MASK_LEN = 0, COVER_MASK_CAUSAL = 1, COVER_MASK_VISLEN = 2 };
```

Result: no change. 961.3 candidates/s (median of 2 runs) (+0.1%).
